# flysoaryun/LF-VIO

Measured on AMD Instinct MI355X. Metric: sliding-window solves/sec (10 KF x N landmarks), higher is better.
Workload: dtype f64; 1 GPU; window300; landmarks=300, observations=1419, windows_per_gpu=1, marginalization=MARGIN_OLD, parallelism=1 independent window stream(s), one per GPU, no data-path collective

## Files before the change

### lf-vio_amd/csrc/dev_types.h

```cpp
#pragma once
#include "../../include/lfvio.h"

constexpr int KC = 73;
constexpr int KP = 172;
constexpr int WLD = 80;
__host__ __device__ inline int w_row_len(int cnt) { return 6 * cnt + 9; }
constexpr int COL_B = 73;
constexpr int COL_K = 74;
constexpr int NQ = 105;
constexpr int NG = 210;
constexpr int NGP = 212;
constexpr int NPAIR = 121;
constexpr int NT = 15;
constexpr int SCHUR_LEN = NT * 256;
constexpr int PACKED = KP * (KP + 1) / 2;
constexpr int JMAX_SWEEPS = 20;
constexpr int PRE_CHUNK_LIMIT = 2 * 121;
constexpr int SUM_ITEMS_CAP = PRE_CHUNK_LIMIT * 209 + 64;
constexpr int SUM_VIS_PACKED = 73 * 74 / 2, SUM_VIS = SUM_VIS_PACKED + 73;
constexpr int HPP_CAP = 16384;
constexpr int XOFF_H = 0;
constexpr int XOFF_G = 14880;
constexpr int XOFF_S = XOFF_G + 176;
constexpr int XOFF_C = XOFF_S + 15 * 256;
constexpr int XCH_LEN = XOFF_C + 16;
constexpr int XP_WGS = 128, XOFF_P = XCH_LEN, XCH_ALLOC = XCH_LEN + 2 * XP_WGS;
enum { XS_COST = 0, XS_G2, XS_ASV2, XS_LAM2, XS_BMAX, XS_GN2, XS_GGN, XS_CCOST, XS_MLIN, XS_MQUAD, XS_DN, XS_XN, XS_N0, XS_ERR };
constexpr int LM_BLOCK = 64;
constexpr int CHUNK_LANES = 64;
constexpr int CHUNK_MAX = 64;
constexpr int SCHUR_LM = 64;
constexpr int LMS = 16;
constexpr int IMU_RAW = 450 + 16;
constexpr int IMU_OUT = 900 + 30 + 2;

__host__ __device__ inline int off_pose(int f) { return 6 * f; }
__host__ __device__ inline int off_ex() { return 66; }
__host__ __device__ inline int off_td() { return 72; }
__host__ __device__ inline int off_sb(int f) { return 73 + 9 * f; }
__host__ __device__ inline int pidx(int i, int j) { return i >= j ? i * (i + 1) / 2 + j : j * (j + 1) / 2 + i; }

struct FrameState {
  double pose[LFVIO_NUM_FRAMES][7];
  double sb[LFVIO_NUM_FRAMES][9];
  double ex[7];
  double td;
};

struct Tab {
  double R[11][9], P[11][3];
  double ric[9], ricT[9], tic[3];
  double M1[11][9];
  double M2[NPAIR][9];
  double T[NPAIR][9];
  double c[NPAIR][3];
};
constexpr int TAB_EX_BIT = 11;
constexpr double TAB_OFF_SPHERE = 1e-14;
__host__ __device__ inline int tab_cj(int pair) { return (pair % 11) * 11 + pair / 11; }

enum {
  Q_GG = 0,
  Q_GN,
  Q_NN,
  Q_gG,
  Q_gN,
  Q_GRAD_SQ,
  Q_GN_SQ,
  Q_GRAD_GN,
  Q_ZG,
  Q_LGN,
  Q_LGG,
  Q_LEX,
  Q_COUNT = 16
};

#ifndef LFVIO_SPEC_EXTRA
#define LFVIO_SPEC_EXTRA 3
#endif
constexpr int SPEC_EXTRA = LFVIO_SPEC_EXTRA, SPEC_MAX_LM = 320;
constexpr int WT_PAIRS = (KC + 1) / 2;
constexpr int SPEC_OWN = 72;
enum { SPEC_FREE = 0, SPEC_SIDE = 1, SPEC_MAIN = 2, SPEC_COMMIT = 3, SPEC_ABANDON = 4 };
enum { FIN_OPEN = 0, FIN_CLOSING = 1, FIN_MAIN = 2, FIN_SIDE = 3 };
constexpr int MAIL_MAX_LM = 8192;
#define TR_HEAD_FIELDS \
  double radius, mu, x_cost, x_norm, cand_cost, model_cost_change, dogleg_step_norm, alpha; \
  double cg, cn; \
  double gn_sq_total, grad_sq_total, grad_gn_total; \
  double step_sq_pose; \
  double xn2_pose_cand; \
  double gmax_pose, lm_bmax; \
  double initial_cost; \
  double function_tolerance; \
  double q[Q_COUNT]; \
  int iteration, cur, do_lin, do_schur, done, termination, chol_fail, scaled; \
  int num_succ, num_unsucc, consec_invalid, trace_len, step_valid, skip_step, error, new_point; \
  int spec_n, gn_unconfirmed;  \
  double cgE[SPEC_EXTRA], cnE[SPEC_EXTRA], snE[SPEC_EXTRA], step_sqE[SPEC_EXTRA], xn2E[SPEC_EXTRA];
struct TRHead {
  TR_HEAD_FIELDS
};
// ... 156 lines not shown
```

### lf-vio_amd/csrc/kernels_lin.h

```cpp
#pragma once
#include "dev_factors.h"
#include "kernels_spec.h"
#include "tr_decide.h"
#include <type_traits>

#define SLOT(base, stride) ((Slot *)((char *)(base) + (size_t)blockIdx.y * (stride)))

constexpr int MODE_SOLVE = 0;
constexpr int MODE_MARG = 1;
constexpr int MODE_GATED = 16;
constexpr int MODE_DECIDE = 64;
constexpr int MODE_NOCOUNT = 32;
DEV bool tail_gate(const Slot *S, int done) { return done && S->tail_state == TAIL_OPEN; }
DEV bool is_marg(int mode) { return mode >= MODE_MARG; }
DEV const MargPlan *marg_plan(const Slot *S, int mode) { return &S->marg[mode - MODE_MARG]; }

DEV int gidx20(int p, int q) { return p * 20 - (p * (p - 1)) / 2 + (q - p); }

constexpr int SETUP_PRIOR_WGS = 16;
constexpr int SETUP_WGS = 2 + SETUP_PRIOR_WGS;
constexpr int SETUP_TILED_MAXN = 88;
__global__ __launch_bounds__(256, 4) void k_setup(char *base, size_t stride, int mode, int zero_wt) {
  Slot *S = SLOT(base, stride);
  const int tid = threadIdx.x;
  constexpr int SETUP_PRIOR_SLAB = 2048, SETUP_LDS = LFVIO_WINDOW_SIZE * 15 * 16;
  static_assert(SETUP_LDS >= SETUP_PRIOR_SLAB + LFVIO_MAX_PRIOR_DIM && SETUP_LDS >= 84 + TAB_SCRATCH, "k_setup's workspace");
  __shared__ double sh_setup[SETUP_LDS];
  const int setup_wgs = (zero_wt & 4) ? 3 : SETUP_WGS;
  if (blockIdx.x == 0) {
    const double *src = (const double *)&S->x0;
    double *dst = (double *)&S->x[0];
    for (int k = tid; k < (int)(sizeof(FrameState) / 8); k += 256) dst[k] = src[k];
    if (tid == 0) {
      TRState *t = &S->tr;
      tr_init(t, S->init_radius, S->fn_tol);
      S->tail_state = TAIL_OPEN;
      S->passes_used = 0;
      S->dec_pending = 0;
      if (mode >= MODE_MARG) t->mu = 0.0;
    }
    double *bt = sh_setup;
    if (tid < 77) bt[tid] = (&S->x0.pose[0][0])[tid];
    else if (tid < 84) bt[tid] = S->x0.ex[tid - 77];
    __syncthreads();
    const unsigned offm = build_tab(bt, &S->tab[0], tid, bt + 84);
    if (tid == 0) S->ex_fixed_off = ((offm >> TAB_EX_BIT) & 1u) && !S->est_ex;
    if (tid == 0 && S->spec_on) spec_arm(S);
  } else if (blockIdx.x == 1) {
    if (tid >= 16 * ((LFVIO_WINDOW_SIZE + 3) & ~3)) return;
    const int grp = tid >> 4, l = tid & 15;
    const int f = grp < LFVIO_WINDOW_SIZE ? grp : 0;
    const bool mine = grp < LFVIO_WINDOW_SIZE && S->imu_active[f];
    const double *cov = S->imu[f].covariance;
    double m0[15], m1[15];
#pragma unroll
    for (int r = 0; r < 15; r++) {
      m0[r] = l < 15 ? cov[r * 15 + l] : (r == 0 ? 1.0 : 0.0);
      m1[r] = r == l + 1 ? 1.0 : 0.0;
    }
#pragma unroll
    for (int k = 0; k < 15; k++) {
      int p = k;
      double best = -1.0, piv = 0.0;
#pragma unroll
      for (int r = 0; r < 15; r++) {
        const double v = fabs(m0[r]);
        if (r >= k && v > best) best = v, p = r, piv = m0[r];
      }
      p = row_bcast_ik(p, k), piv = row_bcast_k(piv, k);
      double csr[15];
#pragma unroll
      for (int r = 0; r < 15; r++) csr[r] = row_bcast_k(m0[r], k);
      const double ck = csr[k];
#pragma unroll
      for (int r = 0; r < 15; r++) csr[r] = r == p ? ck : csr[r];
      auto step = [&](double(&m)[15]) {
        double Mp = m[0];
#pragma unroll
        for (int r = 1; r < 15; r++) Mp = p == r ? m[r] : Mp;
        const double Mk = m[k], mk = Mp / piv;
#pragma unroll
        for (int r = 0; r < 15; r++) {
          const double Msr = r == p ? Mk : m[r];
          m[r] = r == k ? mk : Msr - csr[r] * mk;
        }
      };
      step(m0), step(m1);
    }
    double *T = sh_setup + f * (15 * 16);
// ... 196 lines not shown
  int rows = Nlim - lm0;
  rows = rows > lmb ? lmb : rows;
  auto sweep = [&](auto ntl) {
    constexpr int NTL = decltype(ntl)::value;
    for (int s4 = 0; 4 * s4 < rows; s4++) {
      const int row = 4 * s4 + kk;
      const double coef = lcoef[row], eb = le[row];
#pragma unroll
      for (int j = 0; j < NTL; j++)
        acc[j] = __builtin_amdgcn_mfma_f64_16x16x4f64(coef * tile[row][ct[j]], tile[row][cu[j]] * (scale_k[j] ? eb : 1.0), acc[j], 0, 0, 0);
    }
  };
  if (TIGHT) {
    if (__builtin_amdgcn_readfirstlane(wv) + 12 < NT) sweep(std::integral_constant<int, 4>{});
    else sweep(std::integral_constant<int, 3>{});
  } else {
    for (int s4 = 0; 4 * s4 < rows; s4++) {
      const int row = 4 * s4 + kk;
      const double coef = lcoef[row], eb = le[row];
#pragma unroll
      for (int j = 0; j < 4; j++) {
        if (wv + 4 * j >= NT) continue;
        const double xa = tile[row][ct[j]];
        double xb = tile[row][cu[j]];
        if (mode == MODE_SOLVE && cu[j] == COL_K) xb *= eb;
        acc[j] = __builtin_amdgcn_mfma_f64_16x16x4f64(coef * xa, xb, acc[j], 0, 0, 0);
      }
    }
  }
#pragma unroll
  for (int j = 0; j < 4; j++) {
    if (wv + 4 * j >= NT) continue;
#pragma unroll
    for (int r = 0; r < 4; r++) part[(wv + 4 * j) * 256 + r * 64 + lane] = acc[j][r];
  }
}
DEV int w_col(int ci, int start, int cnt) { return ci < 6 * cnt ? 6 * start + ci : 66 + (ci - 6 * cnt); }

struct LinView {
  const FrameState *x;
  const Tab *tab;
  const double *lam;
  double mu;
};

template <int LPT>
DEV void lin_schur_only_role(Slot *S, const LinView &lv, int wg, double *lds, double *part) {
  constexpr int LMB = LIN_THREADS / LPT;
  double(*tile)[WLD + 1] = (double(*)[WLD + 1]) lds;
  double *lcoef = lds + LM_BLOCK * (WLD + 1) + 64, *le = lcoef + LM_BLOCK;
  const int tid = threadIdx.x;
  for (int e = tid; e < LM_BLOCK * (WLD + 1); e += LIN_THREADS) lds[e] = 0.0;
  __syncthreads();
  {
    const int lml = tid / LPT, q = tid % LPT, l = wg * LMB + lml;
    if (l < S->N) {
      const int st = S->lm_start[l], cnt = S->lm_cnt[l];
      const double *w = S->W + S->lm_woff[l];
      for (int ci = q; ci < w_row_len(cnt); ci += LPT) tile[lml][w_col(ci, st, cnt)] = w[ci];
    }
  }
  if (tid < LM_BLOCK) {
    const int l = wg * LMB + tid;
    double cf = 0.0, eb = 0.0;
    if (tid < LMB && l < S->N) {
      const double sc = S->scale_l[l], s2a = sc * sc * S->a[l];
      const double D2 = fmin(fmax(s2a, 1e-6), 1e32);
      eb = s2a + lv.mu * D2;
      const double einv = 1.0 / eb;
      cf = sc * sc * einv;
      S->einv_l[l] = einv;
    }
    lcoef[tid] = cf, le[tid] = eb;
  }
  __syncthreads();
  schur_block<false>(wg * LMB, LMB, MODE_SOLVE, S->N, tile, lcoef, le, part);
}

#ifdef LFVIO_LIN_PROFILE
#define LSTAMP(k) do { if (blockIdx.x == 0 && mode == MODE_SOLVE && threadIdx.x == 0) S->dbg[k] = (long long)__builtin_readcyclecounter(); } while (0)
#else
#define LSTAMP(k) do { } while (0)
#endif
template <bool TIGHT, int LPT, bool OFFS>
DEV void lin_landmark_role(Slot *S, const LinView &lv, int wg, int mode, double *lds, double *part) {
  constexpr int LMB = LIN_THREADS / LPT;
  double(*tile)[WLD + 1] = (double(*)[WLD + 1]) lds;
  double *red = lds + LM_BLOCK * (WLD + 1);
  double *lcoef = red + 64, *le = lcoef + LM_BLOCK;
  const int tid = threadIdx.x, lml = tid / LPT, q = tid % LPT;
  const TRState *tr = &S->tr;
  const Tab *T = lv.tab;
  const int Nlim = is_marg(mode) ? marg_plan(S, mode)->N0 : S->N;
  const int l = wg * LMB + lml;
  const bool valid = l < Nlim;
  const int est_td = S->est_td;
  const int est_ex = is_marg(mode) ? 1 : S->est_ex;
  const double td = lv.x->td;
  LSTAMP(22);
  for (int e = tid; e < LM_BLOCK * (WLD + 1); e += LIN_THREADS) lds[e] = 0.0;
  if (tid < 2 * LM_BLOCK) lcoef[tid] = 0.0;
  __syncthreads();
  LSTAMP(8);
  double a = 0, b = 0, cost = 0, lam = 1.0, wtd = 0;
  d3 wPi = mk3(0, 0, 0), wTi = wPi, wTic = wPi, wTx = wPi;
  int i = 0, cnt_l = 0, woff_l = 0;
  if (valid) {
    i = S->lm_start[l];
    const int k = S->lm_cnt[l], o0 = S->lm_obs0[l];
    cnt_l = k, woff_l = S->lm_woff[l];
    lam = lv.lam[l];
    ObsPair ob;
    load_obs(S, o0, ob.pi, ob.vi, ob.tdi, ob.rowi);
    const m33 ricT = ldm(T->ricT);
    const unsigned offm = OFFS ? tab_offmask(T) : 0u;
    for (int o = 1 + q; o < k; o += LPT) {
      const int j = i + o, pair = i * 11 + j;
      load_obs(S, o0 + o, ob.pj, ob.vj, ob.tdj, ob.rowj);
      PairU u;
      if (OFFS) load_pair_uniform(T, pair, offm, u);
      else load_pair_uniform(T, pair, u);
      Basis B;
      visual_basis<OFFS>(ob, lam, td, est_td, S->tr_over_row, S->half_row, S->sqrt_info, u, B);
      const double jl0 = B.jl[0], jl1 = B.jl[1];
      d3 eR = jl0 * B.red[0] + jl1 * B.red[1];
      const m33 M1 = ldm(T->M1[j]);
      d3 wp = vmul(eR, M1);
      wPi = wPi + wp;
      wTi = wTi + (jl0 * B.jti[0] + jl1 * B.jti[1]);
      d3 wtj = jl0 * B.jtj[0] + jl1 * B.jtj[1];
      tile[lml][6 * j + 0] = -wp.x, tile[lml][6 * j + 1] = -wp.y, tile[lml][6 * j + 2] = -wp.z;
      tile[lml][6 * j + 3] = wtj.x, tile[lml][6 * j + 4] = wtj.y, tile[lml][6 * j + 5] = wtj.z;
      m33 M3 = u.M2;
#pragma unroll
      for (int e = 0; e < 9; e++) M3.a[e] -= ricT.a[e];
      wTic = wTic + vmul(eR, M3);
      wTx = wTx + (jl0 * B.jtx[0] + jl1 * B.jtx[1]);
      wtd += jl0 * B.jtd[0] + jl1 * B.jtd[1];
      a += jl0 * jl0 + jl1 * jl1;
      b += jl0 * B.r[0] + jl1 * B.r[1];
      cost += 0.5 * B.rho0;
    }
  }
  LSTAMP(9);
  wPi = track_sum3<LPT>(wPi), wTi = track_sum3<LPT>(wTi), wTic = track_sum3<LPT>(wTic), wTx = track_sum3<LPT>(wTx);
  wtd = track_sum<LPT>(wtd), a = track_sum<LPT>(a), b = track_sum<LPT>(b), cost = track_sum<LPT>(cost);
  const bool lead = valid && q == 0;
  if (lead) {
    tile[lml][6 * i + 0] = wPi.x, tile[lml][6 * i + 1] = wPi.y, tile[lml][6 * i + 2] = wPi.z;
    tile[lml][6 * i + 3] = wTi.x, tile[lml][6 * i + 4] = wTi.y, tile[lml][6 * i + 5] = wTi.z;
    if (est_ex) {
      tile[lml][66] = wTic.x, tile[lml][67] = wTic.y, tile[lml][68] = wTic.z;
      tile[lml][69] = wTx.x, tile[lml][70] = wTx.y, tile[lml][71] = wTx.z;
    }
    if (est_td) tile[lml][72] = wtd;
  }
  double g2 = 0, asv2 = 0, lam2 = 0, bmax = 0;
  if (lead) {
    double s = 1.0, D2 = a;
    if (mode == MODE_SOLVE) {
      if (!tr->scaled) {
        s = 1.0 / (1.0 + sqrt(a));
        S->scale_l[l] = s;
      } else {
        s = S->scale_l[l];
      }
      D2 = fmin(fmax(s * s * a, 1e-6), 1e32);
      const double dg = sqrt(D2);
      const double gr = s * b / dg;
      S->diag_l[l] = dg;
      S->grad_l[l] = gr;
      g2 = gr * gr;
      const double v = gr / dg;
      asv2 = s * s * a * v * v;
      tile[lml][COL_K] = b / D2;
      const double s2a = s * s * a;
      const double eb = s2a + lv.mu * D2, einv = 1.0 / eb;
      le[lml] = eb, lcoef[lml] = s * s * einv;
      S->einv_l[l] = einv;
    } else {
      const double cf = (a > 1e-8) ? 1.0 / a : 0.0;
      le[lml] = a, lcoef[lml] = cf;
      S->einv_l[l] = cf;
    }
    S->a[l] = a;
    S->b[l] = b;
    tile[lml][COL_B] = b;
    lam2 = lam * lam;
    bmax = fabs(b);
  } else {
    cost = 0.0;
  }
  LSTAMP(18);
  cost = wave_sum(cost);
  g2 = wave_sum(g2);
  asv2 = wave_sum(asv2);
  lam2 = wave_sum(lam2);
  bmax = wave_max(bmax);
  if ((tid & 63) == 0) {
    double *r = red + 8 * (tid >> 6);
    r[0] = cost, r[1] = g2, r[2] = asv2, r[3] = lam2, r[4] = bmax;
  }
  lds_barrier();
  if (tid < 5) {
    double *p = S->lm_part + (size_t)(LPT == 8 ? wg >> 1 : wg) * LMS + (LPT == 8 && (wg & 1) ? 10 : 0);
    p[tid] = tid < 4 ? ((red[tid] + red[8 + tid]) + (red[16 + tid] + red[24 + tid]))
                     : fmax(fmax(red[4], red[12]), fmax(red[20], red[28]));
  }
  LSTAMP(19);
  if (valid) {
    double *w = S->W + woff_l;
    for (int ci = q; ci < w_row_len(cnt_l); ci += LPT) w[ci] = tile[lml][w_col(ci, i, cnt_l)];
  }
  if (TIGHT && mode == MODE_SOLVE && S->N <= SPEC_MAX_LM) {
    constexpr int WGRP = LIN_THREADS / LMB;
    const int lr = tid % LMB, wg4 = tid / LMB;
    double2 *wt = (double2 *)(double *)S->Wt + wg * LMB + lr;
    constexpr int WPT = (WT_PAIRS + WGRP - 1) / WGRP;
    double2 v[WPT];
#pragma unroll
    for (int k = 0; k < WPT; k++) {
      const int cp = wg4 + WGRP * k, c = cp < WT_PAIRS ? 2 * cp : 0;
      v[k] = make_double2(tile[lr][c], c + 1 < KC ? tile[lr][c + 1] : 0.0);
    }
#pragma unroll
    for (int k = 0; k < WPT; k++) {
      const int cp = wg4 + WGRP * k;
      if (cp < WT_PAIRS) wt[(size_t)cp * SPEC_MAX_LM] = v[k];
    }
  }
  LSTAMP(23);
  schur_block<TIGHT>(wg * LMB, LMB, mode, Nlim, tile, lcoef, le, part);
  LSTAMP(20);
}

template <bool OFFS>
DEV void lin_gram_role(Slot *S, const LinView &lv, int wg, int mode, double *lds) {
  const int wv = threadIdx.x >> 6, lane = threadIdx.x & 63;
  const int chunk = 4 * wg + wv;
  if (chunk >= S->nChunks) return;
  if (is_marg(mode) && chunk >= marg_plan(S, mode)->nChunks0) return;
  double *my = lds + wv * (32 * 17 + 256 + 14 * 20);
  double(*stage)[17] = (double(*)[17]) my;
  double(*Qf)[16] = (double(*)[16])(my + 32 * 17);
  double(*E)[20] = (double(*)[20])(my + 32 * 17 + 256);
  double(*T1)[20] = (double(*)[20]) my;
  const Tab *T = lv.tab;
  const int pair = S->chunk_pair[chunk];
  const int j = pair % 11;
  const int begin = S->chunk_begin[chunk], end = S->chunk_end[chunk];
  const int est_td = S->est_td;
  const double td = lv.x->td;
  PairU u;
  if (OFFS) load_pair_uniform(T, pair, tab_offmask(T), u);
  else load_pair_uniform(T, pair, u);
  for (int e = lane; e < 14 * 20; e += 64) E[0][e] = 0.0;
  for (int e = lane; e < 32 * 17; e += 64) stage[0][e] = 0.0;
  const int idx = begin + lane;
  double c0[14], c1[14];
#pragma unroll
  for (int e = 0; e < 14; e++) c0[e] = c1[e] = 0.0;
  if (idx < end) {
    const int oj = S->pm_obs[idx], l = S->pm_lm[idx];
    const int oi = S->lm_obs0[l];
    const double lam = lv.lam[l];
    ObsPair ob;
    load_obs(S, oi, ob.pi, ob.vi, ob.tdi, ob.rowi);
    load_obs(S, oj, ob.pj, ob.vj, ob.tdj, ob.rowj);
    Basis B;
    visual_basis<OFFS>(ob, lam, td, est_td, S->tr_over_row, S->half_row, S->sqrt_info, u, B);
    c0[0] = B.red[0].x, c0[1] = B.red[0].y, c0[2] = B.red[0].z;
    c1[0] = B.red[1].x, c1[1] = B.red[1].y, c1[2] = B.red[1].z;
    c0[3] = B.jti[0].x, c0[4] = B.jti[0].y, c0[5] = B.jti[0].z;
    c1[3] = B.jti[1].x, c1[4] = B.jti[1].y, c1[5] = B.jti[1].z;
    c0[6] = B.jtj[0].x, c0[7] = B.jtj[0].y, c0[8] = B.jtj[0].z;
    c1[6] = B.jtj[1].x, c1[7] = B.jtj[1].y, c1[8] = B.jtj[1].z;
    c0[9] = B.jtx[0].x, c0[10] = B.jtx[0].y, c0[11] = B.jtx[0].z;
    c1[9] = B.jtx[1].x, c1[10] = B.jtx[1].y, c1[11] = B.jtx[1].z;
    c0[12] = B.jtd[0], c1[12] = B.jtd[1];
    c0[13] = B.r[0], c1[13] = B.r[1];
  }
  double4_t acc = double4_t{0, 0, 0, 0};
  const int nrounds = (end - begin + 15) >> 4;
  for (int r = 0; r < nrounds; r++) {
    __builtin_amdgcn_fence(__ATOMIC_RELEASE, "wavefront");
    if ((lane >> 4) == r) {
      const int row = 2 * (lane & 15);
#pragma unroll
      for (int e = 0; e < 14; e++) stage[row][e] = c0[e], stage[row + 1][e] = c1[e];
    }
    __builtin_amdgcn_fence(__ATOMIC_ACQ_REL, "wavefront");
#pragma unroll
    for (int g = 0; g < 8; g++) {
      const double v = stage[4 * g + (lane >> 4)][lane & 15];
      acc = __builtin_amdgcn_mfma_f64_16x16x4f64(v, v, acc, 0, 0, 0);
    }
  }
  __builtin_amdgcn_fence(__ATOMIC_RELEASE, "wavefront");
#pragma unroll
  for (int r = 0; r < 4; r++) Qf[(lane >> 4) + 4 * r][lane & 15] = acc[r];
  if (lane < 9) {
    const int r = lane / 3, c = lane % 3;
    const double m1 = T->M1[j][lane];
    E[r][c] = m1;
    E[r][6 + c] = -m1;
    E[r][12 + c] = T->M2[pair][lane] - T->ricT[lane];
  } else if (lane < 12) {
    const int k = lane - 9;
    E[3 + k][3 + k] = 1.0;
    E[6 + k][9 + k] = 1.0;
    E[9 + k][15 + k] = 1.0;
  } else if (lane == 12) {
    E[12][18] = 1.0;
    E[13][19] = 1.0;
  }
  __builtin_amdgcn_fence(__ATOMIC_ACQ_REL, "wavefront");
  for (int e = lane; e < 14 * 20; e += 64) {
    const int r = e / 20, c = e % 20;
    double s = 0;
#pragma unroll
    for (int k = 0; k < 14; k++) s = fma(Qf[r][k], E[k][c], s);
    T1[r][c] = s;
  }
  __builtin_amdgcn_fence(__ATOMIC_ACQ_REL, "wavefront");
  double *out = S->gram_part + (size_t)chunk * NGP;
  for (int e = lane; e < 400; e += 64) {
    const int p = e / 20, c = e % 20;
    if (p > c) continue;
    double s = 0;
#pragma unroll
    for (int k = 0; k < 14; k++) s = fma(E[k][p], T1[k][c], s);
    out[gidx20(p, c)] = s;
  }
}

template <bool raw_ready>
DEV void lin_imu_role(Slot *S, const LinView &lv, int f, int mode, double *lds) {
  double(*Jr)[30] = (double(*)[30]) lds;
  double(*Jw)[31] = (double(*)[31])(lds + 450);
  double *rr = lds + 450 + 465, *rw = rr + 16;
  const int tid = threadIdx.x;
  double *out = S->imu_out + (size_t)f * IMU_OUT;
  const bool active = S->imu_active[f] && (mode == MODE_SOLVE || (f == 0 && marg_plan(S, mode)->use_imu0)) &&
                      (!S->sharded || S->pose_side);
  if (!active) {
    for (int e = tid; e < IMU_OUT; e += LIN_THREADS) out[e] = 0.0;
    return;
  }
  const FrameState *x = lv.x;
  if (raw_ready) {
    const double *raw = S->imu_raw + (size_t)f * IMU_RAW;
    for (int e = tid; e < 450; e += LIN_THREADS) Jr[e / 30][e % 30] = raw[e];
    if (tid < 15) rr[tid] = raw[450 + tid];
  } else {
    for (int e = tid; e < 450; e += LIN_THREADS) Jr[e / 30][e % 30] = 0.0;
    __syncthreads();
    if (tid == 0) imu_raw_residual(&S->imu[f], S->g, x->pose[f], x->sb[f], x->pose[f + 1], x->sb[f + 1], rr);
    if (tid == 64) imu_raw_jacobian(&S->imu[f], S->g, x->pose[f], x->sb[f], x->pose[f + 1], x->sb[f + 1], &Jr[0][0]);
  }
  __syncthreads();
  const double *Sq = S->imu_sqrt[f];
  if (tid < 15) {
    double s = 0;
    for (int k = 0; k < 15; k++) s = fma(Sq[tid * 15 + k], rr[k], s);
    rw[tid] = s;
  }
  for (int e = tid; e < 450; e += LIN_THREADS) {
    const int r = e / 30, c = e % 30;
    double s = 0;
    for (int k = r; k < 15; k++) s = fma(Sq[r * 15 + k], Jr[k][c], s);
    Jw[r][c] = s;
  }
  __syncthreads();
  for (int e = tid; e < 900; e += LIN_THREADS) {
    const int p = e / 30, c = e % 30;
    double s = 0;
#pragma unroll
    for (int k = 0; k < 15; k++) s = fma(Jw[k][p], Jw[k][c], s);
    out[e] = s;
  }
  if (tid < 30) {
    double s = 0;
#pragma unroll
    for (int k = 0; k < 15; k++) s = fma(Jw[k][tid], rw[k], s);
    out[900 + tid] = s;
  }
  if (tid == 32) {
    double s = 0;
    for (int k = 0; k < 15; k++) s = fma(rw[k], rw[k], s);
    out[930] = 0.5 * s;
  }
}

template <bool STAGED>
DEV void lin_prior_role(Slot *S, const LinView &lv, int mode, double *lds) {
  const int n = S->prior_n;
  const bool staged = STAGED && n <= LIN_PRIOR_N;
  double *Js = lds, *dx = lds + (STAGED ? LIN_PRIOR_N * LIN_PRIOR_N : 0), *r = dx + KP, *part = r + KP;
  const int tid = threadIdx.x;
  double *g = S->prior_g;
  for (int c = tid; c < KP + 4; c += LIN_THREADS) g[c] = 0.0;
  if (!S->prior_valid || (S->sharded && !S->pose_side)) return;
  const FrameState *x = lv.x;
  const double *Jg = S->prior_J;
  if (staged) {
    constexpr int PER = (LIN_PRIOR_N * LIN_PRIOR_N + LIN_THREADS - 1) / LIN_THREADS;
    double v[PER];
#pragma unroll
    for (int k = 0; k < PER; k++) v[k] = tid + LIN_THREADS * k < n * n ? Jg[tid + LIN_THREADS * k] : 0.0;
    if (tid < S->prior_nb) prior_block_dx(S, x, tid, dx);
#pragma unroll
    for (int k = 0; k < PER; k++)
      if (tid + LIN_THREADS * k < n * n) Js[tid + LIN_THREADS * k] = v[k];
  } else if (tid < S->prior_nb) {
    prior_block_dx(S, x, tid, dx);
  }
  __syncthreads();
  const double *J = staged ? Js : Jg;
  for (int row = tid >> 2; row < n; row += LIN_THREADS / 4) {
    double s = 0;
    for (int c = tid & 3; c < n; c += 4) s = fma(J[row * n + c], dx[c], s);
    s = quad_sum(s);
    if ((tid & 3) == 0) r[row] = S->prior_r[row] + s;
  }
  __syncthreads();
  {
    const int c = tid & 127, h = tid >> 7, k0 = h ? n / 2 : 0, k1 = h ? n : n / 2;
    for (int cc = c; cc < n; cc += 128) {
      double s = 0;
      for (int k = k0; k < k1; k++) s = fma(J[k * n + cc], r[k], s);
      part[h * KP + cc] = s;
    }
  }
  __syncthreads();
  for (int c = tid; c < n; c += LIN_THREADS) g[S->prior_cmap[c]] = part[c] + part[KP + c];
  if (tid < 64) {
    double cs = 0;
    for (int row = tid; row < n; row += 64) cs += r[row] * r[row];
    cs = wave_sum(cs);
    if (tid == 0) g[KP] = 0.5 * cs;
  }
}

__global__ __launch_bounds__(64) void k_imu_raw(char *base, size_t stride, int count) {
  const int g = blockIdx.x * 64 + threadIdx.x;
  if (g >= count * LFVIO_WINDOW_SIZE) return;
  const int slot = g / LFVIO_WINDOW_SIZE, f = g - slot * LFVIO_WINDOW_SIZE;
  Slot *S = reinterpret_cast<Slot *>(base + stride * (size_t)slot);
  const TRFlags fl = tr_flags(&S->tr);
  if (fl.done | !fl.do_lin) return;
  if (!S->imu_active[f] || (S->sharded && !S->pose_side)) return;
  const FrameState *x = &S->x[fl.cur];
  double *raw = S->imu_raw + (size_t)f * IMU_RAW;
  for (int e = 0; e < 450; e++) raw[e] = 0.0;
  imu_raw_residual(&S->imu[f], S->g, x->pose[f], x->sb[f], x->pose[f + 1], x->sb[f + 1], raw + 450);
  imu_raw_jacobian(&S->imu[f], S->g, x->pose[f], x->sb[f], x->pose[f + 1], x->sb[f + 1], raw);
}

constexpr int LIN_ROLE_LM = 1, LIN_ROLE_GRAM = 2, LIN_ROLE_POSE = 4, LIN_ROLE_ALL = 7;
constexpr int LIN_ROLE_POSE_RAW = 8;
constexpr int LIN_LDS_POSE = 1024;
template <int ROLES, bool OFFS = true>
__global__ __launch_bounds__(LIN_THREADS, ROLES == LIN_ROLE_GRAM ? 3 : (ROLES == LIN_ROLE_POSE_RAW ? 6 : 2)) void k_lin(char *base, size_t stride, int mode_bits, int gLw, int gCh) {
  Slot *S = SLOT(base, stride);
  TRState *tr = &S->tr;
  const int mode = mode_bits & (MODE_GATED - 1);
  LSTAMP(21);
  const TRFlags fl = tr_flags(tr);
  int do_lin = fl.do_lin, do_schur = fl.do_schur, cur = fl.cur, acc_z = 0;
  double mu = tr->mu;
  int num_succ = tr->num_succ;
  if (mode_bits & MODE_GATED) {
    if (!tail_gate(S, fl.done)) return;
  } else {
    int done = fl.done;
    const bool owner = blockIdx.x == 0 && !(mode_bits & MODE_NOCOUNT);
    if ((mode_bits & MODE_DECIDE) && !done) {
      __shared__ TRDecision dsh;
      if (threadIdx.x < 64) {
        TRHead t = *reinterpret_cast<const TRHead *>(tr);
        const int K = decide_candidates(t);
        DecideSums sm;
        decide_sums(S, t, K, 0, S->nLmBlocks, threadIdx.x, sm);
        if (threadIdx.x == 0) {
          const int az = decide_walk(t, sm, K, 0, S->max_iter, owner ? tr : nullptr);
          decision_from(dsh, t, az);
          if (owner) S->dec = dsh, S->dec_pending = 1;
        }
      }
      __syncthreads();
      do_lin = __builtin_amdgcn_readfirstlane(dsh.do_lin), do_schur = __builtin_amdgcn_readfirstlane(dsh.do_schur);
      cur = __builtin_amdgcn_readfirstlane(dsh.cur), acc_z = __builtin_amdgcn_readfirstlane(dsh.acc_z), done = __builtin_amdgcn_readfirstlane(dsh.done);
      num_succ = __builtin_amdgcn_readfirstlane(dsh.num_succ);
      mu = __hiloint2double(__builtin_amdgcn_readfirstlane(__double2hiint(dsh.mu)), __builtin_amdgcn_readfirstlane(__double2loint(dsh.mu)));
      if (acc_z > 0 && blockIdx.x == gridDim.x - 1 && !(mode_bits & MODE_NOCOUNT)) {
        copy_accepted(S, acc_z, cur, S->N, threadIdx.x, LIN_THREADS);
        if (S->spec_on) {
          __threadfence();
          __syncthreads();
          if (threadIdx.x == 0) spec_publish(S, num_succ, cur);
        }
      } else if (acc_z == 0 && owner && threadIdx.x == 0 && S->spec_on) spec_publish(S, num_succ, cur);
    } else if (owner && threadIdx.x == 0 && mode == MODE_SOLVE && S->spec_on) spec_publish(S, num_succ, cur);
    if (mode == MODE_SOLVE && owner && !done && threadIdx.x == 0) S->passes_used++;
    if (done | (!do_lin & !do_schur)) return;
  }
  LinView lv;
  lv.x = acc_z > 0 ? &S->xE[acc_z > 0 ? acc_z - 1 : 0] : &S->x[cur];
  lv.tab = acc_z > 0 ? &S->tabE[acc_z > 0 ? acc_z - 1 : 0] : &S->tab[cur];
  lv.lam = acc_z > 0 ? (const double *)S->lamE[acc_z > 0 ? acc_z - 1 : 0] : (const double *)S->lam[cur];
  lv.mu = mu;
  __shared__ __attribute__((aligned(16))) double lds[(ROLES & (LIN_ROLE_LM | LIN_ROLE_GRAM)) ? LIN_LDS : LIN_LDS_POSE];
  int b = blockIdx.x;
  if (b < gLw) {
    if (ROLES & LIN_ROLE_LM) {
      const int half = S->lm_half, lmb = half ? LM_BLOCK / 2 : LM_BLOCK;
      const int nblk = ((is_marg(mode) ? marg_plan(S, mode)->N0 : S->N) + lmb - 1) / lmb;
      if (b >= nblk) return;
      double *part = S->schur_part + (size_t)b * SCHUR_LEN;
      if (half) {
        if (do_lin) lin_landmark_role<ROLES == LIN_ROLE_ALL, 8, OFFS>(S, lv, b, mode, lds, part);
        else lin_schur_only_role<8>(S, lv, b, lds, part);
      } else {
        if (do_lin) lin_landmark_role<ROLES == LIN_ROLE_ALL, 4, OFFS>(S, lv, b, mode, lds, part);
        else lin_schur_only_role<4>(S, lv, b, lds, part);
      }
    }
    return;
  }
  if (!do_lin) return;
  b -= gLw;
  if (b < gCh) {
    if (ROLES & LIN_ROLE_GRAM) lin_gram_role<OFFS>(S, lv, b, mode, lds);
    return;
  }
  b -= gCh;
  if (ROLES & (LIN_ROLE_POSE | LIN_ROLE_POSE_RAW)) {
    if (b < LFVIO_WINDOW_SIZE) {
      if (ROLES & LIN_ROLE_POSE_RAW) lin_imu_role<true>(S, lv, b, mode, lds);
      else lin_imu_role<false>(S, lv, b, mode, lds);
      return;
    }
    lin_prior_role<ROLES == LIN_ROLE_ALL>(S, lv, mode, lds);
  }
}

DEV int schur_index(int R, int Cc) {
  const int t = R >> 4, u = Cc >> 4;
  const int tile = t * 5 - (t * (t - 1)) / 2 + (u - t);
  const int row = R & 15, col = Cc & 15;
  return tile * 256 + (row >> 2) * 64 + ((row & 3) << 4) + col;
}

constexpr int HPP_ITEMS = PACKED + KP;
constexpr int HPP_BLOCKS = (HPP_ITEMS + 255) / 256;

DEV int imu_local(int c, int f) {
  if (c < 66) {
    const int fr = c / 6, l = c - 6 * fr;
    if (fr == f) return l;
    if (fr == f + 1) return 15 + l;
    return -1;
  }
  if (c < KC) return -1;
  const int fr = (c - KC) / 9, l = (c - KC) - 9 * fr;
  if (fr == f) return 6 + l;
  if (fr == f + 1) return 21 + l;
  return -1;
}
DEV int col_frame(int c) { return c < 66 ? c / 6 : (c < KC ? -10 : (c - KC) / 9); }
DEV bool pose_terms_here(const Slot *S, int r) { return !S->sharded || S->pose_side == 1 || (S->pose_side == 2 && r >= KC); }

DEV bool col_active(const Slot *S, int c, int mode) {
  if (mode >= MODE_MARG) return true;
  if (!S->est_ex && c >= off_ex() && c < off_ex() + 6) return false;
  if (!S->est_td && c == off_td()) return false;
  return true;
}

constexpr int PRE_GROUP = 32;
__global__ __launch_bounds__(256) void k_presum(char *base, size_t stride, int mode_bits, int groups) {
  const int PRE_SCHUR_BLOCKS = (SCHUR_LEN / 256) * groups;
  Slot *S = SLOT(base, stride);
  const TRState *tr = &S->tr;
  const int mode = mode_bits & (MODE_GATED - 1);
  const TRFlags fl = tr_flags_decided(S);
  if (mode_bits & MODE_GATED) {
    if (!tail_gate(S, fl.done)) return;
  } else if (fl.done | (!fl.do_lin & !fl.do_schur)) return;
  const int tid = threadIdx.x;
  int b = blockIdx.x;
  if (b < NPAIR) {
    if (!fl.do_lin) return;
    const int chunk_limit = is_marg(mode) ? marg_plan(S, mode)->nChunks0 : S->nChunks;
    const int c0 = S->pair_chunk0[b];
    int c1 = S->pair_chunk0[b + 1];
    if (c1 > chunk_limit) c1 = chunk_limit;
    if (tid < NGP) {
      const double *gp = S->gram_part + tid;
      double s0 = 0, s1 = 0, s2 = 0, s3 = 0;
      int c = c0;
      for (; c + 4 <= c1; c += 4) {
        s0 += gp[(size_t)c * NGP], s1 += gp[(size_t)(c + 1) * NGP];
        s2 += gp[(size_t)(c + 2) * NGP], s3 += gp[(size_t)(c + 3) * NGP];
      }
      for (; c < c1; c++) s0 += gp[(size_t)c * NGP];
      S->pairG[(size_t)b * NGP + tid] = (s0 + s1) + (s2 + s3);
    }
    return;
  }
  b -= NPAIR;
  if (b < PRE_SCHUR_BLOCKS) {
    if (!fl.do_schur) return;
    const int grp = b / (SCHUR_LEN / 256), e = (b % (SCHUR_LEN / 256)) * 256 + tid;
    int parts = S->nSchurParts;
    if (is_marg(mode)) parts = (marg_plan(S, mode)->N0 + S->schur_lm - 1) / S->schur_lm;
    const int p0 = grp * PRE_GROUP;
    if (p0 >= parts) return;
    const int p1 = min(parts, p0 + PRE_GROUP);
    double *sp = S->schur_part + e;
    double a0 = 0, a1 = 0, a2 = 0, a3 = 0;
    int p = p0;
    for (; p + 4 <= p1; p += 4) {
      a0 += sp[(size_t)p * SCHUR_LEN], a1 += sp[(size_t)(p + 1) * SCHUR_LEN];
      a2 += sp[(size_t)(p + 2) * SCHUR_LEN], a3 += sp[(size_t)(p + 3) * SCHUR_LEN];
    }
    for (; p < p1; p++) a0 += sp[(size_t)p * SCHUR_LEN];
    sp[(size_t)p0 * SCHUR_LEN] = (a0 + a1) + (a2 + a3);
    return;
  }
  if (!fl.do_lin) return;
  __shared__ double red[5][256];
  const int blocks = S->nLmBlocks;
  double v[5] = {0, 0, 0, 0, 0};
  for (int k = tid; k < blocks; k += 256) {
    const double *q = S->lm_part + (size_t)k * LMS;
    v[0] += q[0], v[1] += q[1], v[2] += q[2], v[3] += q[3], v[4] = fmax(v[4], q[4]);
  }
#pragma unroll
  for (int k = 0; k < 5; k++) red[k][tid] = v[k];
  __syncthreads();
  for (int w = 128; w > 0; w >>= 1) {
    if (tid < w) {
#pragma unroll
      for (int k = 0; k < 4; k++) red[k][tid] += red[k][tid + w];
      red[4][tid] = fmax(red[4][tid], red[4][tid + w]);
    }
    __syncthreads();
  }
  if (tid < 5) S->lm_sum[tid] = red[tid][0];
}

struct SumArgs {
  long long sum_off, sum_end_marg, sum_items, gram_part, pairG, imu_out, prior_A;
};
template <class T>
DEV T *blob_at(const Slot *S, long long off) { return (T *)((char *)S + off); }
#define SUM_KEEP(v) asm volatile("" ::"v"(v))

DEV void sum_hpp_entry(Slot *S, const SumArgs &o, int mode_bits, int e) {
  const int mode = mode_bits & (MODE_GATED - 1);
  const bool in = e < HPP_ITEMS;
  const int ec = in ? e : 0;
  const bool packed = ec < PACKED;
  int r, c;
  if (packed) {
    r = (int)((sqrt(8.0 * ec + 1.0) - 1.0) * 0.5);
    while ((r + 1) * (r + 2) / 2 <= ec) r++;
    while (r * (r + 1) / 2 > ec) r--;
    c = ec - r * (r + 1) / 2;
  } else {
    r = c = ec - PACKED;
  }
  const TRFlags fl = tr_flags_decided(S);
  const int tail_state = S->tail_state, est_ex = S->est_ex, est_td = S->est_td, prior_valid = S->prior_valid, sharded = S->sharded;
  const int pose_side = S->pose_side, pre_gram = S->pre_gram, prior_n = S->prior_n;
  const int marg_chunks = is_marg(mode) ? marg_plan(S, mode)->nChunks0 : 1;
  const int vis = r < KC ? (packed ? ec : SUM_VIS_PACKED + r) : 0;
  const int beg = blob_at<int>(S, o.sum_off)[vis];
  int end = blob_at<int>(S, o.sum_off)[vis + 1];
  const int endm = blob_at<int>(S, o.sum_end_marg)[vis];
  const int pr = S->prior_inv[r], pc = S->prior_inv[c];
  const double pg = S->prior_g[r];
  double imu_v[2] = {0.0, 0.0};
  const int f0 = col_frame(r);
  const double *imu_out = blob_at<double>(S, o.imu_out);
#pragma unroll
  for (int u = 0; u < 2; u++) {
    const int f = f0 - 1 + u;
    if (f0 >= 0 && f >= 0 && f < LFVIO_WINDOW_SIZE) {
      const int pl = imu_local(r, f), ql = imu_local(c, f);
      if (packed) {
        if (pl >= 0 && ql >= 0) imu_v[u] = imu_out[(size_t)f * IMU_OUT + pl * 30 + ql];
      } else if (pl >= 0) {
        imu_v[u] = imu_out[(size_t)f * IMU_OUT + 900 + pl];
      }
    }
  }
  SUM_KEEP(beg);
  SUM_KEEP(end);
  SUM_KEEP(endm);
  SUM_KEEP(pr);
  SUM_KEEP(pc);
  SUM_KEEP(pg);
  SUM_KEEP(imu_v[0]);
  SUM_KEEP(imu_v[1]);
  if (mode_bits & MODE_GATED) {
    if (!(fl.done && tail_state == TAIL_OPEN)) return;
  } else if (fl.done | !fl.do_lin) return;
  if (!in) return;
  const bool act_r = is_marg(mode) || !((!est_ex && r >= off_ex() && r < off_ex() + 6) || (!est_td && r == off_td()));
  const bool act_c = is_marg(mode) || !((!est_ex && c >= off_ex() && c < off_ex() + 6) || (!est_td && c == off_td()));
  double val = 0.0;
  if (act_r && act_c) {
    if (is_marg(mode)) end = marg_chunks > 0 ? endm : beg;
    const bool pterms = !sharded || pose_side == 1 || (pose_side == 2 && r >= KC);
    const bool use_prior = packed && prior_valid && pterms && pr >= 0 && pc >= 0;
    double pa = 0.0;
    if (use_prior) pa = blob_at<double>(S, o.prior_A)[pr * prior_n + pc];
    if (r < KC) {
      const int *it = blob_at<int>(S, o.sum_items);
      const double *gp = blob_at<double>(S, pre_gram ? o.pairG : o.gram_part);
      double s0 = 0, s1 = 0, s2 = 0, s3 = 0;
      int k = beg;
      for (; k + 4 <= end; k += 4) {
        const int o0 = it[k], o1 = it[k + 1], o2 = it[k + 2], o3 = it[k + 3];
        s0 += gp[o0], s1 += gp[o1], s2 += gp[o2], s3 += gp[o3];
      }
      for (; k < end; k++) s0 += gp[it[k]];
      val += (s0 + s1) + (s2 + s3);
    }
    if (packed) {
      if (f0 >= 0 && pterms) {
#pragma unroll
        for (int u = 0; u < 2; u++) {
          const int f = f0 - 1 + u;
          if (f >= 0 && f < LFVIO_WINDOW_SIZE && imu_local(r, f) >= 0 && imu_local(c, f) >= 0) val += imu_v[u];
        }
      }
      if (use_prior) val += pa;
// ... 104 lines not shown
```

### lf-vio_amd/csrc/kernels_linw.h

```cpp
#pragma once
#include "kernels_lin.h"

#ifdef LFVIO_LINW_PROFILE
#ifndef LFVIO_LINB_GROUP
#define LFVIO_LINB_GROUP 0
#endif
#define WSTAMP(k) do { if (blockIdx.y == 0 && threadIdx.x == 0) S->dbg[k] = (long long)__builtin_readcyclecounter(); } while (0)
#define WACC(k, t0) do { wacc[(k) - 24] += (long long)__builtin_readcyclecounter() - (t0); } while (0)
#define WNOW() ((long long)__builtin_readcyclecounter())
#else
#define WSTAMP(k) do { } while (0)
#define WACC(k, t0) do { } while (0)
#define WNOW() 0ll
#endif

constexpr int LW_THREADS = 256;
constexpr int LW_STAGE = 32 * 17;
constexpr int LW_WAVE = LW_STAGE + 256 + 64;
constexpr int LW_D = 0, LW_FX = 11 * 21, LW_XX = LW_FX + 11 * 42, LW_G = LW_XX + 28, LW_DUMMY = LW_G + 76;
constexpr int LW_PRIV = 800;
static_assert(LW_DUMMY < LW_PRIV, "private accumulator layout");
constexpr int LW_NPAIR = 55, LW_OFF = LW_NPAIR * 36;
constexpr int LW_PRIV0 = LINW_WAVES * LW_WAVE, LW_OFF0 = LW_PRIV0 + LINW_WAVES * LW_PRIV, LW_RED0 = LW_OFF0 + LW_OFF;
constexpr int LW_LDS_P1 = LW_RED0 + LINW_WAVES * 8;
// ... 328 lines not shown
  auto factor_on = [&](int f) { return S->imu_active[f] && pose_rank && (mode == MODE_SOLVE || (f == 0 && marg_plan(S, mode)->use_imu0)); };
  for (int e = lane; e < 3 * 16 * LW_JLD; e += 64) my[e] = 0.0;
  __builtin_amdgcn_fence(__ATOMIC_ACQ_REL, "wavefront");
  if (lane < 3) {
    const int f = wv + 4 * lane;
    if (f < LFVIO_WINDOW_SIZE && factor_on(f)) {
      double rr[15];
      imu_raw_residual(&S->imu[f], S->g, x->pose[f], x->sb[f], x->pose[f + 1], x->sb[f + 1], rr);
      double *Jr = Jr3 + 16 * LW_JLD * lane;
#pragma unroll
      for (int k = 0; k < 15; k++) Jr[k * LW_JLD + 30] = rr[k];
      imu_raw_jacobian(&S->imu[f], S->g, x->pose[f], x->sb[f], x->pose[f + 1], x->sb[f + 1], Jr, LW_JLD);
    }
  }
  __builtin_amdgcn_fence(__ATOMIC_ACQ_REL, "wavefront");
  WSTAMP(29);
  const int kq = lane >> 4, ii = lane & 15;
  double *imu_out = (double *)((char *)S + imu_off);
  double sa3[3][4];
#pragma unroll
  for (int q = 0; q < 3; q++) {
    const int f = wv + 4 * q < LFVIO_WINDOW_SIZE ? wv + 4 * q : 0;
    const double *Sq = S->imu_sqrt[f];
#pragma unroll
    for (int s4 = 0; s4 < 4; s4++) {
      const int k = 4 * s4 + kq;
      sa3[q][s4] = (ii < 15 && k < 15) ? Sq[ii * 15 + k] : 0.0;
    }
  }
#pragma unroll
  for (int q = 0; q < 3; q++) {
    const int f = wv + 4 * q;
    if (f >= LFVIO_WINDOW_SIZE) break;
    double *out = imu_out + (size_t)f * IMU_OUT;
    if (!factor_on(f)) {
      for (int e = lane; e < IMU_OUT; e += 64) out[e] = 0.0;
      continue;
    }
    const double(*Jr)[LW_JLD] = (const double(*)[LW_JLD])(Jr3 + 16 * LW_JLD * q);
    const double(&sa)[4] = sa3[q];
    double4_t w0 = double4_t{0, 0, 0, 0}, w1 = w0;
#pragma unroll
    for (int s4 = 0; s4 < 4; s4++) {
      w0 = __builtin_amdgcn_mfma_f64_16x16x4f64(sa[s4], Jr[4 * s4 + kq][ii], w0, 0, 0, 0);
      w1 = __builtin_amdgcn_mfma_f64_16x16x4f64(sa[s4], Jr[4 * s4 + kq][16 + ii], w1, 0, 0, 0);
    }
#pragma unroll
    for (int r = 0; r < 4; r++) Jw[kq + 4 * r][ii] = w0[r], Jw[kq + 4 * r][16 + ii] = w1[r];
    __builtin_amdgcn_fence(__ATOMIC_ACQ_REL, "wavefront");
    double4_t g00 = double4_t{0, 0, 0, 0}, g01 = g00, g11 = g00;
#pragma unroll
    for (int s4 = 0; s4 < 4; s4++) {
      const double v0 = Jw[4 * s4 + kq][ii], v1 = Jw[4 * s4 + kq][16 + ii];
      g00 = __builtin_amdgcn_mfma_f64_16x16x4f64(v0, v0, g00, 0, 0, 0);
      g01 = __builtin_amdgcn_mfma_f64_16x16x4f64(v0, v1, g01, 0, 0, 0);
      g11 = __builtin_amdgcn_mfma_f64_16x16x4f64(v1, v1, g11, 0, 0, 0);
    }
#pragma unroll
    for (int r = 0; r < 4; r++) {
      const int row = kq + 4 * r, c1 = 16 + ii;
      auto ord = [](int p) { return p < 6 ? p : p < 15 ? p + 6 : p < 21 ? p - 9 : p; };
      const int r2 = 16 + row;
      if (ord(row) >= ord(ii)) out[row * 30 + ii] = g00[r];
      if (c1 < 30) {
        if (ord(row) >= ord(c1)) out[row * 30 + c1] = g01[r];
        else out[c1 * 30 + row] = g01[r];
      } else if (c1 == 30) out[900 + row] = g01[r];
      if (r2 < 30) {
        if (c1 < 30) {
          if (ord(r2) >= ord(c1)) out[r2 * 30 + c1] = g11[r];
        } else if (c1 == 30) out[900 + r2] = g11[r];
      } else if (r2 == 30 && c1 == 30) out[930] = 0.5 * g11[r];
    }
    __builtin_amdgcn_fence(__ATOMIC_ACQ_REL, "wavefront");
  }
}

constexpr int LW_PRIOR_MAXN = 88;
static_assert(LW_PRIOR_MAXN * LW_PRIOR_MAXN + 4 * KP <= LW_LDS_P1, "prior stage fits");
DEV void linw_prior(Slot *S, const LinView &lv, double *lw) {
  const int tid = threadIdx.x;
  const int n = S->prior_n;
  if (!S->prior_valid || (S->sharded && !S->pose_side) || n > LW_PRIOR_MAXN) {
    lin_prior_role<false>(S, lv, MODE_SOLVE, lw);
    __syncthreads();
    return;
  }
  double *Js = lw, *dx = lw + LW_PRIOR_MAXN * LW_PRIOR_MAXN, *r = dx + KP, *part = r + KP;
  double *g = S->prior_g;
  const double *J = S->prior_J;
  const double r0_row = (tid >> 1) < n ? S->prior_r[tid >> 1] : 0.0;
  const int cmap_c = tid < n ? S->prior_cmap[tid] : 0;
  {
    constexpr int PJ = 8, ROUNDS = (LW_PRIOR_MAXN * LW_PRIOR_MAXN + PJ * LW_THREADS - 1) / (PJ * LW_THREADS);
    const int nn = n * n;
#pragma unroll 1
    for (int b = 0; b < ROUNDS && b * PJ * LW_THREADS < nn; b++) {
      double v[PJ];
#pragma unroll
      for (int k = 0; k < PJ; k++) {
        const int e = tid + LW_THREADS * (PJ * b + k);
        v[k] = J[e < nn ? e : 0];
      }
#pragma unroll
      for (int k = 0; k < PJ; k++) {
        const int e = tid + LW_THREADS * (PJ * b + k);
        if (e < nn) Js[e] = v[k];
      }
    }
  }
  for (int c = tid; c < KP + 4; c += LW_THREADS) g[c] = 0.0;
  if (tid < S->prior_nb) prior_block_dx(S, lv.x, tid, dx);
  __syncthreads();
  {
    const int row = tid >> 1, h = tid & 1;
    double s0 = 0, s1 = 0, s2 = 0, s3 = 0;
    if (row < n) {
      const double *jr = Js + row * n;
      int c = h;
      for (; c + 6 < n; c += 8) s0 = fma(jr[c], dx[c], s0), s1 = fma(jr[c + 2], dx[c + 2], s1), s2 = fma(jr[c + 4], dx[c + 4], s2), s3 = fma(jr[c + 6], dx[c + 6], s3);
      for (; c < n; c += 2) s0 = fma(jr[c], dx[c], s0);
    }
    double sum = (s0 + s1) + (s2 + s3);
    sum += dpp_f64<0xB1>(sum);
    if (row < n && h == 0) r[row] = r0_row + sum;
  }
  __syncthreads();
  {
    const int c = tid & 127, h = tid >> 7, k0 = h ? n / 2 : 0, k1 = h ? n : n / 2;
    if (c < n) {
      double s0 = 0, s1 = 0, s2 = 0, s3 = 0;
      int k = k0;
      for (; k + 3 < k1; k += 4)
        s0 = fma(Js[k * n + c], r[k], s0), s1 = fma(Js[(k + 1) * n + c], r[k + 1], s1), s2 = fma(Js[(k + 2) * n + c], r[k + 2], s2), s3 = fma(Js[(k + 3) * n + c], r[k + 3], s3);
      for (; k < k1; k++) s0 = fma(Js[k * n + c], r[k], s0);
      part[h * KP + c] = (s0 + s1) + (s2 + s3);
    }
  }
  __syncthreads();
  static_assert(LW_PRIOR_MAXN <= LW_THREADS, "one column per thread");
  if (tid < n) g[cmap_c] = part[tid] + part[KP + tid];
  if (tid < 64) {
    double cs = 0;
    for (int row = tid; row < n; row += 64) cs += r[row] * r[row];
    cs = wave_sum(cs);
    if (tid == 0) g[KP] = 0.5 * cs;
  }
  __syncthreads();
}

constexpr int LWT_ABS = 1 << 16, LWT_EX = 1 << 17, LWT_TD = 1 << 18;

template <bool OFFS>
DEV void linw_body(Slot *S, double *lw, const LinwArgs &A, int mode_bits) {
  TRState *tr = &S->tr;
  const int tid = threadIdx.x, wv = tid >> 6, lane = tid & 63;
  TRFlags fl = tr_flags(tr);
  const double mu = tr->mu;
  const int mode = mode_bits & (MODE_GATED - 1);
  const bool marg = is_marg(mode);
  const int N = marg ? marg_plan(S, mode)->N0 : S->N, est_ex = marg ? 1 : S->est_ex, est_td = marg ? 1 : S->est_td;
  if (marg) {
    if ((mode_bits & MODE_GATED) && !tail_gate(S, fl.done)) return;
    fl.do_lin = fl.do_schur = 1;
  } else {
    if (!fl.done && tid == 0) S->passes_used++;
    if (fl.done | (!fl.do_lin & !fl.do_schur)) return;
// ... 160 lines not shown
  double *einv_l = lw_at<double>(S, A.einv_l);
  const int nblk = (N + LM_BLOCK - 1) / LM_BLOCK;
  constexpr int WPT = (WT_PAIRS + 3) / 4;
  double2 wreg[WPT];
  double w_sc = 0, w_a = 0, w_b = 0;
  auto request = [&](int blk) {
    const int l = blk * LM_BLOCK + lane;
    const int pmin = 3 * rfl(blk_start[blk]);
#pragma unroll
    for (int k = 0; k < WPT; k++) {
      const int cp = wv + 4 * k;
      wreg[k] = (cp < WT_PAIRS && cp >= pmin && l < N) ? wt0[(size_t)cp * SPEC_MAX_LM + l] : make_double2(0.0, 0.0);
    }
    if (tid < LM_BLOCK && l < N) w_sc = scale_l[l], w_a = av[l], w_b = bv[l];
  };
  for (int e = tid; e < LM_BLOCK * 6; e += LW_THREADS) tile[e / 6][75 + e % 6] = 0.0;
  if (nblk > 0) request(0);
  for (int blk = 0; blk < nblk; blk++) {
    __syncthreads();
    {
      const int l = blk * LM_BLOCK + lane;
#pragma unroll
      for (int k = 0; k < WPT; k++) {
        const int cp = wv + 4 * k;
        if (cp < WT_PAIRS) {
          tile[lane][2 * cp] = wreg[k].x;
          if (2 * cp + 1 < KC) tile[lane][2 * cp + 1] = wreg[k].y;
        }
      }
      if (tid < LM_BLOCK) {
        double cf = 0.0, eb = 0.0, bl = 0.0, kap = 0.0;
        if (l < N && marg) {
          cf = (w_a > 1e-8) ? 1.0 / w_a : 0.0, eb = w_a, bl = w_b;
        } else if (l < N) {
          const double s2a = w_sc * w_sc * w_a;
          const double D2 = fmin(fmax(s2a, 1e-6), 1e32);
          eb = s2a + mu * D2;
          const double einv = 1.0 / eb;
          cf = w_sc * w_sc * einv;
          if (!fl.do_lin) einv_l[l] = einv;
          bl = w_b, kap = bl / D2;
        }
        lcoef[tid] = cf, le[tid] = eb;
        tile[tid][COL_B] = bl, tile[tid][COL_K] = kap;
      }
    }
    if (blk + 1 < nblk) request(blk + 1);
    __syncthreads();
    auto sweep = [&](auto ntl) {
      constexpr int NTL4 = decltype(ntl)::value;
#pragma unroll
      for (int s4 = 0; s4 < LM_BLOCK / 4; s4++) {
        const int row = 4 * s4 + kk;
        const double coef = lcoef[row], eb = le[row];
#pragma unroll
        for (int j = 0; j < NTL4; j++) {
          const double xa = tile[row][ct[j]];
          double xb = tile[row][cu[j]];
          if (scale_k[j]) xb *= eb;
          acc[j] = __builtin_amdgcn_mfma_f64_16x16x4f64(coef * xa, xb, acc[j], 0, 0, 0);
        }
      }
    };
    if (__builtin_amdgcn_readfirstlane(wv) + 12 < NT) sweep(std::integral_constant<int, 4>{});
    else sweep(std::integral_constant<int, 3>{});
  }
  WSTAMP(13);
  double *ss = lw_at<double>(S, A.schur_sum);
#pragma unroll
  for (int j = 0; j < 4; j++) {
    if (wv + 4 * j >= NT) continue;
#pragma unroll
    for (int r = 0; r < 4; r++) ss[(wv + 4 * j) * 256 + r * 64 + lane] = acc[j][r];
  }
  if (tid == 0 && !marg && fl.do_lin) S->wt_clean = 1;
  WSTAMP(14);
}
template <bool OFFS = true>
__global__ __launch_bounds__(LW_THREADS, 2) void k_linw(char *base, size_t stride, const LinwArgs A, int mode_bits) {
  extern __shared__ __attribute__((aligned(16))) double lw[];
  linw_body<OFFS>(SLOT(base, stride), lw, A, mode_bits);
}

constexpr int LINB_LEN = SUM_VIS + SCHUR_LEN + 8;
__global__ __launch_bounds__(256) void k_linb_gather(char *base, size_t stride) {
  Slot *S = SLOT(base, stride);
  if (!S->linw.big) return;
  const int i = blockIdx.x * 256 + threadIdx.x;
  if (i < S->N) {
    const int o = S->lm_obs0[i];
#pragma unroll
    for (int k = 0; k < 8; k++) S->anc[k][i] = S->obs[k][o];
  }
  if (i < S->NV) {
    const int o = S->pm_obs[i];
    double v[8];
#pragma unroll
    for (int k = 0; k < 8; k++) v[k] = S->obs[k][o];
#pragma unroll
    for (int k = 0; k < 8; k++) S->pmo[k][i] = v[k];
    int lo = 0, hi = NPAIR;
    while (hi - lo > 1) {
      const int mid = (lo + hi) >> 1;
      if (S->linw.pair_obs0[mid] <= i) lo = mid;
      else hi = mid;
    }
    S->pm_pair[i] = (unsigned char)lo;
  }
}
#ifdef LFVIO_LINW_PROFILE
#ifndef LFVIO_LINB_GROUP
#define LFVIO_LINB_GROUP 0
#endif
#define BSTAMP(k) do { if (blockIdx.x == LFVIO_LINB_GROUP && blockIdx.y == 0 && threadIdx.x == 0) S->dbg[k] = (long long)__builtin_readcyclecounter(); } while (0)
#else
#define BSTAMP(k) do { } while (0)
#endif
template <bool OFFS>
DEV void linb_body(Slot *S, double *lw, const LinwArgs &A) {
  TRState *tr = &S->tr;
  const int tid = threadIdx.x, wv = tid >> 6, lane = tid & 63;
  const TRFlags fl = tr_flags(tr);
  const double mu = tr->mu;
  const LinwPlan *P = &S->linw;
  const int ng = P->ng, g = blockIdx.x;
  if (g > ng) return;
  if (g == 0 && tid == 0 && !fl.done) S->passes_used++;
  if (fl.done | (!fl.do_lin & !fl.do_schur)) return;
  LinView lv;
  lv.x = &S->x[fl.cur], lv.tab = &S->tab[fl.cur], lv.lam = lw_at<const double>(S, A.lam[fl.cur]), lv.mu = mu;
  if (g == ng) {
    if (!fl.do_lin) return;
    linw_imu(S, lv, lw, A.imu_out, MODE_SOLVE);
    __syncthreads();
    linw_prior(S, lv, lw);
    return;
  }
  const int L0 = rfl(S->linb_lm0[g]), ns = rfl(S->linb_ns[g]), s = ns >> 16, L1 = L0 + (ns & 0xffff);
  const int est_ex = S->est_ex, est_td = S->est_td;
  double *out = lw_at<double>(S, A.part) + (size_t)g * LINB_LEN;
  if (fl.do_lin) {
    constexpr int P3_E = (SUM_VIS + LW_THREADS - 1) / LW_THREADS;
    int p3[P3_E];
#pragma unroll
    for (int q = 0; q < P3_E; q++) p3[q] = A.asm_tab[tid + LW_THREADS * q < SUM_VIS ? tid + LW_THREADS * q : 0];
    const int nstr = (L1 - L0 + LM_BLOCK - 1) / LM_BLOCK, split = nstr <= 1 ? 4 : nstr <= 2 ? 2 : 1;
    const int mine = wv / split + (lane == 1 ? 4 : 0);
    const int lm0w = L0 + LM_BLOCK * mine, nw = min(max(L1 - lm0w, 0), LM_BLOCK);
    const int kmaxw = nw > 0 ? S->lm_cnt[lm0w + nw - 1] : 0;
    const int nmine = (wv / split < nstr ? 1 : 0) + (wv / split + 4 < nstr ? 1 : 0);
    BSTAMP(8);
    for (int e = tid; e < LB_RED0 + LINW_WAVES * 8; e += LW_THREADS) lw[e] = 0.0;
    __syncthreads();
    BSTAMP(9);
    double part[5];
    linw_strips<true, OFFS>(S, lv, A, fl.cur, fl.scaled, MODE_SOLVE, lw, part, 0, nmine, lm0w, nw | (s << 8) | (kmaxw << 16), 1 + wv % split, split);
    if (lane == 0) {
#pragma unroll
      for (int k = 0; k < 5; k++) lw[LB_RED0 + 8 * wv + k] = part[k];
    }
    __syncthreads();
    BSTAMP(10);
#pragma unroll
    for (int q = 0; q < P3_E; q++) {
      const int e = tid + LW_THREADS * q, d = p3[q];
      int at = d & 0xffff;
      bool live = true;
// ... 246 lines not shown
```

### lf-vio_amd/csrc/kernels_marg.h

```cpp
#pragma once
#include "kernels_solve.h"

constexpr int MARG_THREADS = 768;
constexpr int MARG_MAXD = 96;
constexpr int LDN = 80;
constexpr double JACOBI_TOL = 1e-19;
constexpr size_t MARG_LDS = (size_t)19072 * sizeof(double);
constexpr int BT_GROUP = 4;

DEV void gauge_landmarks(Slot *S, int l0) {
  const int l = l0 + (int)threadIdx.x;
  double *lam = S->lam[S->tr.cur];
  if (l < S->N) lam[l] = 1.0 / (1.0 / lam[l]);
}
template <class T>
DEV void copy_rounds(T *dst, const T *src, int n, int tid, int nthr) {
  for (int k0 = tid; k0 < n; k0 += 8 * nthr) {
    T v[8];
#pragma unroll
    for (int q = 0; q < 8; q++) v[q] = src[k0 + q * nthr < n ? k0 + q * nthr : 0];
#pragma unroll
    for (int q = 0; q < 8; q++)
      if (k0 + q * nthr < n) dst[k0 + q * nthr] = v[q];
  }
// ... 118 lines not shown
  if (!tail_gate(S, S->tr.done)) return;
  const int spec = S->spec_on;
  if (spec) {
    if (threadIdx.x == 0) spec_closing(S);
    __syncthreads();
  }
  {
    constexpr int LT = (SPEC_MAX_LM + 127) / 128;
    double *lam = S->lam[S->tr.cur];
    const int N = S->N, tid = threadIdx.x;
    double lv[LT];
#pragma unroll
    for (int k = 0; k < LT; k++) lv[k] = lam[tid + 128 * k < N ? tid + 128 * k : 0];
#pragma unroll
    for (int k = 0; k < LT; k++)
      if (tid + 128 * k < N) lam[tid + 128 * k] = 1.0 / (1.0 / lv[k]);
    for (int l0 = 128 * LT; l0 < N; l0 += 128) gauge_landmarks(S, l0);
  }
  gauge_poses(S, 1, publish != 0);
  if (spec && threadIdx.x == 0) spec_settle(S);
}
DEV void gauge_poses(Slot *S, int gated, bool publish) {
  TRState *ts = &S->tr;
  const int tid = threadIdx.x;
  __shared__ double rot[9], P0[3], oP0[3];
  FrameState *x = &S->x[ts->cur];
  if (tid == 0) {
    const m33 Rs0 = q2R(q_from_pose(S->x0.pose[0]));
    const m33 R00 = q2R(q_from_pose(x->pose[0]));
    const double h0 = sqrt(Rs0.a[0] * Rs0.a[0] + Rs0.a[3] * Rs0.a[3]), h00 = sqrt(R00.a[0] * R00.a[0] + R00.a[3] * R00.a[3]);
    const double c0 = Rs0.a[0] / h0, s0 = Rs0.a[3] / h0, c00 = R00.a[0] / h00, s00 = R00.a[3] / h00;
    const double cyd = c0 * c00 + s0 * s00, syd = s0 * c00 - c0 * s00;
    m33 rd;
    rd.a[0] = cyd, rd.a[1] = -syd, rd.a[2] = 0;
    rd.a[3] = syd, rd.a[4] = cyd, rd.a[5] = 0;
    rd.a[6] = 0, rd.a[7] = 0, rd.a[8] = 1;
    const double sin1deg = 0.017452406437283512;
    if (h0 < sin1deg || h00 < sin1deg) rd = mm(Rs0, tr(R00));
    for (int k = 0; k < 9; k++) rot[k] = rd.a[k];
    for (int k = 0; k < 3; k++) P0[k] = x->pose[0][k], oP0[k] = S->x0.pose[0][k];
  }
  __syncthreads();
  const m33 rd = ldm(rot);
  d3 Psi = mk3(0, 0, 0), Vsi = Psi;
  q4 qn = q4{1, 0, 0, 0};
  if (tid < 11) {
    const m33 Rsi = mm(rd, q2R(qnormalized(q_from_pose(x->pose[tid]))));
    Psi = mul(rd, ld3(x->pose[tid]) - ld3(P0)) + ld3(oP0);
    Vsi = mul(rd, ld3(x->sb[tid]));
    qn = R2q(Rsi);
  } else if (tid == 11) {
    qn = R2q(q2R(q_from_pose(x->ex)));
  }
  __syncthreads();
  __shared__ double bt[84 + TAB_SCRATCH];
  if (tid < 11) {
    const double pn[7] = {Psi.x, Psi.y, Psi.z, qn.x, qn.y, qn.z, qn.w};
#pragma unroll
    for (int k = 0; k < 7; k++) x->pose[tid][k] = pn[k], bt[7 * tid + k] = pn[k];
    x->sb[tid][0] = Vsi.x, x->sb[tid][1] = Vsi.y, x->sb[tid][2] = Vsi.z;
  } else if (tid == 11) {
    x->ex[3] = qn.x, x->ex[4] = qn.y, x->ex[5] = qn.z, x->ex[6] = qn.w;
#pragma unroll
    for (int k = 0; k < 3; k++) bt[77 + k] = x->ex[k];
    bt[80] = qn.x, bt[81] = qn.y, bt[82] = qn.z, bt[83] = qn.w;
  }
  __syncthreads();
  if (publish) publish_solution(S);
  if (tid == 0) {
    if (!gated) ts->done = 0;
    ts->do_lin = 1;
    ts->do_schur = 1;
    ts->chol_fail = 0;
  }
  build_tab(bt, &S->tab[ts->cur], tid, bt + 84);
}

__global__ __launch_bounds__(64) void k_spec_wait(char *base) {
  Slot *S = (Slot *)base;
  if (threadIdx.x != 0) return;
  const long long t0 = wall_clock64();
  while (spec_peek(&S->tail_state) == TAIL_WORKER && wall_clock64() - t0 < 10 * SPEC_WAIT_TICKS) __builtin_amdgcn_s_sleep(8);
}
__global__ __launch_bounds__(128) void k_spec_begin(char *base, size_t back) {
  Slot *S = (Slot *)base;
  Slot *S0 = (Slot *)(base - back);
  const int tid = threadIdx.x;
  __shared__ int sh_word, sh_go;
  const long long t0 = wall_clock64();
  for (;;) {
    if (tid == 0) {
      int go = 0, w = 0;
      const int last = S->shadow.last_word;
      for (;;) {
        const int f = spec_peek(&S0->spec.fin);
        w = spec_peek(&S0->spec.word);
        if (w != 0) {
          const int st = spec_ep(f) == spec_ep(w) ? spec_fin_state(f) : FIN_OPEN;
          if (st != FIN_OPEN) break;
          if (w != last) {
            go = 1;
            break;
          }
        }
        if (wall_clock64() - t0 > SPEC_WAIT_TICKS) break;
        __builtin_amdgcn_s_sleep(8);
      }
      spec_acquire();
      sh_word = w, sh_go = go;
    }
    __syncthreads();
    int go = __builtin_amdgcn_readfirstlane(sh_go);
    const int w = __builtin_amdgcn_readfirstlane(sh_word);
    if (!go) {
      if (tid == 0) S->shadow.word = 0, S->tr.done = 0;
      return;
    }
    const int ep = spec_ep(w), a = spec_acc(w), cur = w & 1;
    if (S->shadow.hdr_ep != ep) {
      const long long *src = (const long long *)S0;
      long long *dst = (long long *)S;
      constexpr int W0 = (int)(offsetof(Slot, lm_start) / 8), W1 = (int)(offsetof(Slot, x) / 8);
      static_assert(offsetof(Slot, lm_start) % 8 == 0 && offsetof(Slot, x) % 8 == 0, "header words");
      for (int k = tid; k < W1; k += 128) dst[k] = src[k] - (k >= W0 ? (long long)back : 0ll);
      const double *is = &S0->imu_sqrt[0][0];
      double *id = &S->imu_sqrt[0][0];
      for (int k = tid; k < LFVIO_WINDOW_SIZE * 225; k += 128) id[k] = is[k];
    }
    __syncthreads();
    {
      constexpr int XW = (int)(sizeof(FrameState) / 8), TW = (int)(sizeof(TRHead) / 8), XT = (XW + 127) / 128, LT = (SPEC_MAX_LM + 127) / 128;
      static_assert(TW <= 128, "the trust-region header in one trip");
      const double *xs = (const double *)&S0->x[cur];
      double *xd = (double *)&S->x[0];
      const double *ls = S0->lam[cur];
      double *ld = S->lam[0];
      const int N = S0->N;
      const long long *ts = (const long long *)&S0->tr;
      long long *td = (long long *)&S->tr;
      double xv[XT], lv[LT];
#pragma unroll
      for (int k = 0; k < XT; k++) xv[k] = xs[tid + 128 * k < XW ? tid + 128 * k : 0];
#pragma unroll
      for (int k = 0; k < LT; k++) lv[k] = ls[tid + 128 * k < N ? tid + 128 * k : 0];
      const long long tv = ts[tid < TW ? tid : 0];
#pragma unroll
      for (int k = 0; k < XT; k++)
        if (tid + 128 * k < XW) xd[tid + 128 * k] = xv[k];
#pragma unroll
      for (int k = 0; k < LT; k++)
        if (tid + 128 * k < N) ld[tid + 128 * k] = 1.0 / (1.0 / lv[k]);
      if (tid < TW) td[tid] = tv;
      for (int k = tid + 128 * LT; k < N; k += 128) ld[k] = 1.0 / (1.0 / ls[k]);
    }
    __syncthreads();
    if (tid == 0) {
      const int f = spec_ld(&S0->spec.fin), w2 = spec_ld(&S0->spec.word);
      const bool open = spec_ep(f) != ep || spec_fin_state(f) == FIN_OPEN;
      sh_go = (w2 == w && open && spec_cas(&S0->spec.own[a], SPEC_FREE, SPEC_SIDE) == SPEC_FREE) ? 1 : 0;
      S->shadow.hdr_ep = ep;
      S->shadow.last_word = w;
    }
    __syncthreads();
    go = __builtin_amdgcn_readfirstlane(sh_go);
    if (!go) {
      __syncthreads();
      continue;
    }
    if (tid == 0) {
      S->shadow.word = w, S->shadow.ticket = S0->spec.ticket;
      S->spec_on = 0, S->dec_pending = 0, S->tail_state = TAIL_OPEN, S->chain_err = 0;
      S->tr.cur = 0, S->tr.done = 1;
    }
    __syncthreads();
    break;
  }
  gauge_poses(S, 1, false);
}

DEV bool spd_inverse_wave(const double *Am, double *Xout, int m, int lane, double floor) {
  double a[15];
#pragma unroll
  for (int j = 0; j < 15; j++) a[j] = (lane < m && j < m) ? Am[lane * m + j] : (lane == j ? 1.0 : 0.0);
  bool ok = true;
  double dinv = 1.0;
#pragma unroll
  for (int j = 0; j < 15; j++) {
    const double d = readlane_f64(a[j], j);
    ok = ok && (d > 0.0);
    const double rs = fast_rsqrt(d);
    const double l = lane == j ? d * rs : a[j] * rs;
    a[j] = l;
    dinv = lane == j ? rs : dinv;
#pragma unroll
    for (int c = j + 1; c < 15; c++) a[c] = fma(-l, readlane_f64(l, c), a[c]);
  }
  double y[15];
#pragma unroll
  for (int i = 0; i < 15; i++) {
    double t = lane == i ? 1.0 : 0.0;
#pragma unroll
    for (int k = 0; k < i; k++) t = fma(-readlane_f64(a[k], i), y[k], t);
    y[i] = t * readlane_f64(dinv, i);
  }
  double fro = 0;
#pragma unroll
  for (int r = 0; r < 15; r++) {
    double x = 0;
#pragma unroll
    for (int i = r; i < 15; i++) x = fma(readlane_f64(y[i], r), y[i], x);
    if (lane < m && r < m) Xout[r * m + lane] = x, fro += x * x;
  }
  fro = wave_sum(fro);
  return ok && fro * floor * floor < 1.0;
}

DEV void rr_pair(int k, int step, int np, int n, int &p, int &q) {
  if (k == 0) {
    p = step, q = np - 1;
  } else {
    p = step + k;
    if (p >= np - 1) p -= np - 1;
    q = step - k;
    if (q < 0) q += np - 1;
  }
  if (q >= n) q = -1;
}
// ... 784 lines not shown
```

### lf-vio_amd/csrc/lfvio_hip.hip

```cpp
#include <hip/hip_runtime.h>
#include <dlfcn.h>
typedef struct ncclComm *ncclComm_t;
#define NCCL_UNIQUE_ID_BYTES 128
typedef struct {
  char internal[NCCL_UNIQUE_ID_BYTES];
} ncclUniqueId;
typedef int ncclResult_t;
typedef int ncclDataType_t;
typedef int ncclRedOp_t;
constexpr ncclResult_t ncclSuccess = 0;
constexpr ncclRedOp_t ncclSum = 0;
constexpr ncclDataType_t ncclDouble = 8;

#include <algorithm>
#include <chrono>
#include <cmath>
#include <cstdio>
#include <cstdlib>
#include <cstring>
#include <memory>
#include <string>
#include <type_traits>
#include <vector>

#include "../../include/lfvio.h"
#include "../../include/lfvio_debug.h"
#include "kernels_marg.h"
#include "kernels_solve.h"
#include "kernels_feat.h"
#include "kernels_linw.h"
#include "linb_plan.h"
#include "call_state.h"
#include "kernels_stepw.h"
#include "kernels_relo.h"
#include "kernels_twoview.h"
#include "kernels_vialign.h"
#include "kernels_pnp.h"

#define HIPCHK(ctx, call)                                                                      \
  do {                                                                                         \
    hipError_t e_ = (call);                                                                    \
    if (e_ != hipSuccess) {                                                                    \
      (ctx)->err = std::string(#call) + ": " + hipGetErrorString(e_);                          \
      return LFVIO_ERR_DEVICE;                                                                 \
    }                                                                                          \
  } while (0)

namespace {

inline size_t align_up(size_t v, size_t a) { return (v + a - 1) / a * a; }

struct Layout {
  int maxN = 0, maxM = 0;
  int capLmBlocks = 0, capChunks = 0, capSchurParts = 0;
  size_t in_begin = 0, in_end = 0, total = 0;
  size_t anc[8], pmo[8], pm_pair, linb_lm0, linb_ns, linw_begin = 0, linw_end = 0;
  size_t lm_start, lm_cnt, lm_obs0, lm_perm, lm_woff, lam0, obs[8], pm_obs, pm_lm, chunk_pair, chunk_begin, chunk_end, sum_off, sum_end_marg, sum_items, prior_J,
      prior_r;
  size_t lam[2], lamE[SPEC_EXTRA], cost_partE, prior_A, a, b, W, Wt, scale_l, grad_l, gn_l, diag_l, einv_l, d1, d2, gram_part, pairG, schur_part,
      xch, lm_part, cost_part, imu_out, imu_raw, mscr, eig_aux;
};

Layout make_layout(int maxN, int maxM) {
  Layout L;
  L.maxN = maxN;
  L.maxM = maxM;
  L.capLmBlocks = std::max(1, (maxN + LM_BLOCK - 1) / LM_BLOCK);
  L.capChunks = 64 + maxM / CHUNK_MAX;
  L.capSchurParts = std::max(L.capLmBlocks + 1, 2 * ((std::min(maxN, SPEC_MAX_LM) + LM_BLOCK - 1) / LM_BLOCK));
  static_assert(LINB_LEN >= SCHUR_LEN, "the Schur partials of k_lin share the array of k_linb's group partials, which are the larger");
  size_t o = align_up(sizeof(Slot), 256);
  auto take = [&](size_t bytes) {
    size_t r = o;
    o = align_up(o + bytes, 256);
    return r;
  };
  const size_t N = std::max(maxN, 1), M = std::max(maxM, 1), LB = (size_t)L.capLmBlocks * LM_BLOCK;
  L.in_begin = o;
  L.lm_start = take(N * 4), L.lm_cnt = take(N * 4), L.lm_obs0 = take(N * 4), L.lm_perm = take(N * 4);
  L.lm_woff = take((N + 1) * 4);
  L.lam0 = take(N * 8);
  for (int k = 0; k < 8; k++) L.obs[k] = take(M * 8);
  L.pm_obs = take(M * 4), L.pm_lm = take(M * 4);
  L.chunk_pair = take((size_t)L.capChunks * 4), L.chunk_begin = take((size_t)L.capChunks * 4),
  L.chunk_end = take((size_t)L.capChunks * 4);
  L.prior_r = take(LFVIO_MAX_PRIOR_DIM * 8);
  L.sum_off = take((size_t)(SUM_VIS + 1) * 4), L.sum_end_marg = take((size_t)SUM_VIS * 4);
  L.sum_items = take((size_t)SUM_ITEMS_CAP * 4);
  L.prior_J = take((size_t)LFVIO_MAX_PRIOR_DIM * LFVIO_MAX_PRIOR_DIM * 8);
  L.in_end = o;
  L.linw_begin = o;
  for (int k = 0; k < 8; k++) L.anc[k] = take(N * 8);
  for (int k = 0; k < 8; k++) L.pmo[k] = take(M * 8);
  L.pm_pair = take(M);
  L.linb_lm0 = take(((size_t)L.capLmBlocks + LFVIO_NUM_FRAMES + 1) * 4), L.linb_ns = take(((size_t)L.capLmBlocks + LFVIO_NUM_FRAMES + 1) * 4);
  L.linw_end = o;
  L.lam[0] = take(LB * 8), L.lam[1] = take(LB * 8);
  for (int k = 0; k < SPEC_EXTRA; k++) L.lamE[k] = take((size_t)SPEC_MAX_LM * 8);
  L.cost_partE = take((size_t)SPEC_EXTRA * (SPEC_MAX_LM / 64) * LMS * 8);
  L.prior_A = take((size_t)LFVIO_MAX_PRIOR_DIM * LFVIO_MAX_PRIOR_DIM * 8);
  L.a = take(LB * 8), L.b = take(LB * 8), L.W = take(LB * WLD * 8);
  L.Wt = take((size_t)WT_PAIRS * std::max((size_t)SPEC_MAX_LM, LB) * 16);
  L.scale_l = take(LB * 8), L.grad_l = take(LB * 8), L.gn_l = take(LB * 8), L.diag_l = take(LB * 8);
  L.einv_l = take(LB * 8), L.d1 = take(LB * 8), L.d2 = take(LB * 8);
  L.gram_part = take((size_t)L.capChunks * NGP * 8);
  L.pairG = take((size_t)NPAIR * NGP * 8);
  L.schur_part = take((size_t)L.capSchurParts * LINB_LEN * 8);
  L.xch = take((size_t)XCH_ALLOC * 8);
  L.lm_part = take((size_t)L.capLmBlocks * LMS * 8);
  L.cost_part = take((size_t)L.capLmBlocks * LMS * 8);
  L.imu_out = take((size_t)LFVIO_WINDOW_SIZE * IMU_OUT * 8);
  L.imu_raw = take((size_t)LFVIO_WINDOW_SIZE * IMU_RAW * 8);
  L.mscr = take((size_t)HPP_CAP * 8);
  L.eig_aux = take(4096);
  L.total = align_up(o, 4096);
  return L;
}

size_t down_bytes(int maxN) { return sizeof(FrameState) * 2 + sizeof(TRState) + 2 * ((size_t)maxN * 8 + 128) + sizeof(LfvioPrior) + 4096; }

struct SlotHostInfo {
  bool spec_on = false;
  bool offs_first = false, offs_all = false;
  int N = 0, M = 0, gLm = 0, gLw = 0, gCh = 0, gSc = 0;
  int marg_n = 0;
  int prior_n = 0;
  int max_iter = 0;
  double max_seconds = -1.0;
  std::vector<int> perm;
  bool linw_ok = false;
  bool linb_ok = false;
  int linb_ng = 0;
  bool uploaded = false;
  bool resident = false;
  LfvioPrior in_prior;
  bool has_in_prior = false;
  bool in_prior_device = false;
  struct MargOut {
    int valid = 0, n = 0, m = 0, nb = 0;
    int kind[LFVIO_MAX_PRIOR_BLOCKS], frame[LFVIO_MAX_PRIOR_BLOCKS], idx[LFVIO_MAX_PRIOR_BLOCKS];
  } marg_out[2];
  int mail_seq = 0;
  std::vector<int> list_key;
  int list_items = -1;
};

struct Grid {
  int lm, ch, sc, lw;
  int ch_raw;
};

struct SetupLaunch {
  int gx, bits;
};

struct Route {
  enum Sweep { ROLES = 0, LINW = 1, LINB = 2 } sweep;
  int count;
  Grid g;
  size_t role_wgs;
  bool split;
  int linb_gx;
  SetupLaunch setup;
  int offs;
};

struct GraphKey {
  int count = 0, lm = 0, ch = 0, sc = 0, sweep = -1, linb_gx = 0, offs = 0, setup = -1, spec = 0, passes = 0;
  bool operator==(const GraphKey &o) const {
    return count == o.count && lm == o.lm && ch == o.ch && sc == o.sc && sweep == o.sweep && linb_gx == o.linb_gx && offs == o.offs &&
           setup == o.setup && spec == o.spec && passes == o.passes;
  }
};

}

struct lfvio_ctx {
  int device = 0;
  hipStream_t stream = nullptr;
  char *d_feat = nullptr;
  size_t feat_bytes = 0;
  char *h_feat = nullptr;
  std::string err;
  int batch = 0;
  Layout L;
  char *d_base = nullptr;
  char *h_stage = nullptr;
  char *h_down = nullptr;
  size_t h_down_bytes = 0;
  std::vector<SlotHostInfo> info;
  std::vector<int> perm_build;
  hipGraphExec_t graph = nullptr;
  GraphKey graph_key;
  hipGraphExec_t chunk[2] = {}, tail[2][3] = {};
  hipGraphExec_t first[2][2][4][13] = {};
  int fixed_passes = 0;
  int recent_passes[4] = {0, 0, 0, 0}, recent_head = 0;
  int predict_passes = 4;
  double pass_seconds = 2e-4;
  GraphKey chunk_key;
// ... 753 lines not shown

template <class F>
int capture_graph(lfvio_ctx *c, hipStream_t stream, hipGraphExec_t *out, F &&enqueue) {
  hipGraph_t graph;
  HIPCHK(c, hipStreamBeginCapture(stream, hipStreamCaptureModeThreadLocal));
  CaptureGuard guard(stream);
  if (int rc = enqueue()) return rc;
  HIPCHK(c, guard.end(&graph));
  HIPCHK(c, hipGraphInstantiate(out, graph, nullptr, nullptr, 0));
  HIPCHK(c, hipGraphDestroy(graph));
  return LFVIO_OK;
}

constexpr int CH_BUCKET = 16;

Grid grid_for(lfvio_ctx *c, int count) {
  Grid g{1, 1, 1, 1, 1};
  for (int s = 0; s < count; s++) {
    g.ch_raw = std::max(g.ch_raw, c->info[s].gCh);
    g.lm = std::max(g.lm, c->info[s].gLm);
    g.lw = std::max(g.lw, c->info[s].gLw);
    g.ch = std::max(g.ch, c->info[s].gCh);
    g.sc = std::max(g.sc, c->info[s].gSc);
  }
  g.ch = (g.ch + CH_BUCKET - 1) / CH_BUCKET * CH_BUCKET;
  return g;
}

int slots_offs(const lfvio_ctx *c, int count) {
  int r = 0;
  for (int k = 0; k < count; k++) r |= (c->info[k].offs_first ? 1 : 0) | (c->info[k].offs_all ? 2 : 0);
  return r;
}

SetupLaunch setup_launch(lfvio_ctx *c, int count, int lm, bool zero_wt) {
  bool compact = count >= 8;
  for (int s = 0; compact && s < count; s++) compact = c->info[s].prior_n <= SETUP_TILED_MAXN;
  return {(compact ? 3 : SETUP_WGS) + (lm + 3) / 4, (zero_wt ? 1 : 0) | (compact ? 4 : 0)};
}

Route route_for(lfvio_ctx *c, int count, int mode) {
  Route r;
  r.count = count;
  r.g = grid_for(c, count);
  r.role_wgs = (size_t)count * (r.g.lw + (r.g.ch + 3) / 4 + LFVIO_WINDOW_SIZE + 1);
  r.split = count >= LIN_SPLIT_MIN_BATCH && r.role_wgs > LIN_SPLIT_WGS;
  bool linw = true, linb = count > 0;
  int ng = 0;
  for (int s = 0; s < count; s++) {
    linw = linw && c->info[s].linw_ok, linb = linb && c->info[s].linb_ok;
    ng = std::max(ng, c->info[s].linb_ng);
  }
  const bool solve = mode == MODE_SOLVE;
  const bool marg_sweep = (mode & (MODE_GATED - 1)) >= MODE_MARG && !(mode & (MODE_DECIDE | MODE_NOCOUNT));
  if (c->linw_mode != 0 && !c->shard_active && linw && (solve || marg_sweep) && (c->linw_mode == 2 || r.split)) r.sweep = Route::LINW;
  else if (c->linw_mode != 0 && solve && linb && (!c->shard_active || count == 1)) r.sweep = Route::LINB;
  else r.sweep = Route::ROLES;
  r.linb_gx = r.sweep == Route::LINB ? (ng + 1 + 63) / 64 * 64 : 0;
  r.setup = setup_launch(c, count, r.g.lm, r.sweep == Route::LINW);
  r.offs = slots_offs(c, count);
  return r;
}

GraphKey graph_key(const Route &r, int spec, int passes, bool with_setup) {
  GraphKey k;
  k.count = r.count, k.lm = r.g.lm, k.ch = r.g.ch, k.sc = r.g.sc, k.sweep = r.sweep, k.linb_gx = r.linb_gx, k.offs = r.offs;
  k.setup = with_setup ? r.setup.bits : 0, k.spec = spec, k.passes = passes;
  return k;
}

void launch_setup(lfvio_ctx *c, const Route &r, int mode) {
  hipLaunchKernelGGL(k_setup, dim3(r.setup.gx, r.count), dim3(256), 0, c->stream, c->d_base, c->L.total, mode, r.setup.bits);
}

template <class F>
void with_offs(bool offs, F &&launch) {
  if (offs) launch(std::true_type());
  else launch(std::false_type());
}

void launch_lin(lfvio_ctx *c, const Route &r, int mode, bool offs) {
  const int count = r.count, lw = r.g.lw, gram_wgs = (r.g.ch + 3) / 4;
  const size_t st = c->L.total;
  with_offs(offs, [&](auto o) {
    if (!r.split) {
      hipLaunchKernelGGL((k_lin<LIN_ROLE_ALL, decltype(o)::value>), dim3(lw + gram_wgs + LFVIO_WINDOW_SIZE + 1, count), dim3(LIN_THREADS), 0, c->stream, c->d_base, st,
                         mode, lw, gram_wgs);
      return;
    }
    hipLaunchKernelGGL((k_lin<LIN_ROLE_LM, decltype(o)::value>), dim3(lw, count), dim3(LIN_THREADS), 0, c->stream, c->d_base, st, mode, lw, 0);
    hipLaunchKernelGGL((k_lin<LIN_ROLE_GRAM, decltype(o)::value>), dim3(gram_wgs, count), dim3(LIN_THREADS), 0, c->stream, c->d_base, st, mode | MODE_NOCOUNT, 0, gram_wgs);
  });
  if (!r.split) return;
  const bool raw = (mode & (MODE_GATED - 1)) == MODE_SOLVE && !(mode & (MODE_GATED | MODE_DECIDE));
  if (raw) hipLaunchKernelGGL(k_imu_raw, dim3((count * LFVIO_WINDOW_SIZE + 63) / 64), dim3(64), 0, c->stream, c->d_base, st, count);
  if (raw) hipLaunchKernelGGL((k_lin<LIN_ROLE_POSE_RAW, false>), dim3(LFVIO_WINDOW_SIZE + 1, count), dim3(LIN_THREADS), 0, c->stream, c->d_base, st, mode | MODE_NOCOUNT, 0, 0);
  else hipLaunchKernelGGL((k_lin<LIN_ROLE_POSE, false>), dim3(LFVIO_WINDOW_SIZE + 1, count), dim3(LIN_THREADS), 0, c->stream, c->d_base, st, mode | MODE_NOCOUNT, 0, 0);
}

void launch_sum(lfvio_ctx *c, const Route &r, int mode) {
  const int count = r.count;
  const Grid &g = r.g;
  const size_t st = c->L.total;
  const int pre = (g.ch_raw > PRE_CHUNK_LIMIT || g.sc > 4 * PRE_GROUP) ? 1 : 0;
  const int groups = (g.sc + PRE_GROUP - 1) / PRE_GROUP;
  if (pre) hipLaunchKernelGGL(k_presum, dim3(NPAIR + (SCHUR_LEN / 256) * groups + 1, count), dim3(256), 0, c->stream, c->d_base, st, mode, groups);
  const Layout &L = c->L;
  const SumArgs sa{(long long)L.sum_off, (long long)L.sum_end_marg, (long long)L.sum_items, (long long)L.gram_part, (long long)L.pairG, (long long)L.imu_out,
                   (long long)L.prior_A};
  hipLaunchKernelGGL(k_sum, dim3(HPP_BLOCKS + SCHUR_LEN / 256 + 1, count), dim3(256), 0, c->stream, c->d_base, st, mode, pre, sa);
}

LinwArgs linw_args(const lfvio_ctx *c) {
  const Layout &L = c->L;
  LinwArgs a;
  a.anc0 = (long long)L.anc[0], a.anc_stride = (long long)(L.anc[1] - L.anc[0]);
  a.pmo0 = (long long)L.pmo[0], a.pmo_stride = (long long)(L.pmo[1] - L.pmo[0]);
  a.Wt = (long long)L.Wt, a.lam[0] = (long long)L.lam[0], a.lam[1] = (long long)L.lam[1];
  a.a = (long long)L.a, a.b = (long long)L.b, a.scale_l = (long long)L.scale_l, a.diag_l = (long long)L.diag_l, a.grad_l = (long long)L.grad_l;
  a.einv_l = (long long)L.einv_l, a.imu_out = (long long)L.imu_out;
  a.Hpp = (long long)(L.xch + (size_t)XOFF_H * 8), a.gp = (long long)(L.xch + (size_t)XOFF_G * 8), a.schur_sum = (long long)(L.xch + (size_t)XOFF_S * 8);
  a.part = (long long)L.schur_part, a.wt_ld = L.capLmBlocks * LM_BLOCK;
  a.asm_tab = c->d_lwt;
  return a;
}

void launch_sweep(lfvio_ctx *c, const Route &r, int mode, bool offs, bool decide = false) {
  if (r.sweep == Route::ROLES) {
    launch_lin(c, r, mode | (decide ? MODE_DECIDE : 0), offs);
    launch_sum(c, r, mode);
    return;
  }
  const size_t st = c->L.total;
  with_offs(offs, [&](auto o) {
    if (r.sweep == Route::LINW)
      hipLaunchKernelGGL(k_linw<decltype(o)::value>, dim3(1, r.count), dim3(LW_THREADS), LW_LDS_BYTES, c->stream, c->d_base, st, linw_args(c), mode);
    else
      hipLaunchKernelGGL(k_linb<decltype(o)::value>, dim3(r.linb_gx, r.count), dim3(LW_THREADS), LW_LDS_BYTES, c->stream, c->d_base, st, linw_args(c));
  });
  if (r.sweep == Route::LINB) hipLaunchKernelGGL(k_sumb, dim3(LINB_SUM_GRID, r.count), dim3(LINB_SUM_THREADS), 0, c->stream, c->d_base, st, linw_args(c));
}

void launch_solve(lfvio_ctx *c, int count, bool lw = false) {
  const size_t st = c->L.total;
  const long long xo = (long long)c->L.xch, io = (long long)c->L.imu_out, po = (long long)c->L.prior_A;
  if (lw)
    hipLaunchKernelGGL(k_solve_dense<true>, dim3(1, count), dim3(SOLVE_THREADS), SOLVE_LDS, c->stream, c->d_base, st, xo, io, po, (const int *)c->d_asm);
  else
    hipLaunchKernelGGL(k_solve_dense<false>, dim3(1, count), dim3(SOLVE_THREADS), SOLVE_LDS, c->stream, c->d_base, st, xo, io, po, (const int *)nullptr);
}

struct Pass {
  bool speculate = false;
  bool first = true, last = true;
  bool gauge = false;
  bool publish = false;
  bool offs = true;
};
bool launch_iteration(lfvio_ctx *c, const Route &r, int mode, const Pass &ps) {
  const int count = r.count;
  const Grid &g = r.g;
  const size_t st = c->L.total;
  const bool solve = (mode & (MODE_GATED - 1)) == MODE_SOLVE && !(mode & MODE_GATED);
  const bool lw = r.sweep == Route::LINW, lb = r.sweep == Route::LINB;
  const bool merge = solve && !lw && g.lm <= DOGLEG_INLINE_BLOCKS && r.role_wgs <= LIN_SPLIT_WGS;
  launch_sweep(c, r, mode, ps.offs, merge && !ps.first);
  if ((mode & (MODE_GATED - 1)) == MODE_SOLVE) {
    launch_solve(c, count, lw);
    const bool inl = g.lm <= DOGLEG_INLINE_BLOCKS;
    const int spec = ps.speculate && inl ? c->spec_count : 1;
    const int nb = g.lm + LFVIO_WINDOW_SIZE + 1;
    const bool split = r.split || lw;
    const bool fuse = inl && !split && !c->shard_active && (size_t)count * nb <= 2048;
    const bool stepw = lw && inl && spec == 1;
    if (stepw) {
      hipLaunchKernelGGL(k_stepw, dim3(1, count), dim3(STEPW_LAUNCH_THREADS), 0, c->stream, c->d_base, st);
      return false;
    }
    if (!inl && lb) hipLaunchKernelGGL(k_backsub_wt, dim3(g.lm, count), dim3(64), 0, c->stream, c->d_base, st, c->L.capLmBlocks * LM_BLOCK);
    else if (!inl) hipLaunchKernelGGL(k_backsub, dim3(g.lm, count), dim3(64), 0, c->stream, c->d_base, st);
// ... 53 lines not shown
  HIPCHK(c, hipGraphLaunch(graph, c->stream));
  if (int rc = behind()) return rc;
  *early = watch && wait_early(c);
  return LFVIO_OK;
}
void record_mailbox_call(lfvio_ctx *c, unsigned act) {
  record_call(c, *mail_word(c, MAIL_STATE_PASSES), ((const TRState *)(c->h_mail + MAIL_TR))->iteration, act);
}

struct LoopGraphs {
  int first_passes = 0;
  hipGraphExec_t first = nullptr, chunk = nullptr;
};
int loop_graphs(lfvio_ctx *c, const Route &r, const CallPlan &p, int passes, LoopGraphs *G) {
  const int count = r.count;
  const Grid &g = r.g;
  const bool speculate = (size_t)count * (g.lm + LFVIO_WINDOW_SIZE + 1) <= 512;
  if (speculate && !c->fixed_spec) c->spec_count = (c->last_iters > 0 && c->last_iters >= 2 * c->last_passes) ? std::min(4, 1 + SPEC_EXTRA) : 3;
  if (!c->d_pending) {
    HIPCHK(c, hipMalloc((void **)&c->d_pending, 256));
    HIPCHK(c, hipHostMalloc((void **)&c->h_pending, 256, hipHostMallocDefault));
  }
  const int offs = r.offs;
  const GraphKey key = graph_key(r, (int)speculate, 0, true);
  if (!(c->chunk_key == key)) {
    destroy_graph(c, c->chunk_key.count == count && ((c->chunk_key.offs ^ offs) & 2) == 0);
    c->chunk_key = key;
  }
  const bool fuse = p.fused;
  int first_passes = std::min(std::max(c->fixed_passes > 0 ? c->fixed_passes : c->predict_passes, 1), std::min(passes, MAX_FIRST_PASSES));
  if (p.max_seconds > 0.0) first_passes = std::max(std::min(SOLVE_CHUNK, passes), std::min(first_passes, (int)std::min(p.max_seconds / c->pass_seconds, 1e6)));
  G->first_passes = first_passes;
  const int sv = speculate && c->spec_count > 3 ? 1 : 0;
  hipGraphExec_t &first_graph = c->first[sv][p.publish ? 1 : 0][fuse ? 1 + p.marg_flag : 0][first_passes];
  enum Head { PASSES_ONLY, SETUP_FIRST };
  auto capture = [&](hipGraphExec_t *out, Head head, int npass, bool tail) {
    const bool setup = head == SETUP_FIRST;
    return capture_graph(c, c->stream, out, [&]() -> int {
      if (setup) launch_setup(c, r, MODE_SOLVE);
      bool gauged = false;
      Pass ps;
      ps.speculate = speculate, ps.gauge = tail, ps.publish = p.publish;
      for (int it = 0; it < npass; it++) {
        ps.first = it == 0, ps.last = it == npass - 1, ps.offs = (offs & 2) || (setup && it == 0 && (offs & 1));
        gauged = launch_iteration(c, r, MODE_SOLVE, ps);
      }
      if (tail) {
        if (!gauged) {
          hipLaunchKernelGGL(k_gauge, dim3(1 + (g.lm + 1) / 2, count), dim3(128), 0, c->stream, c->d_base, c->L.total, 1);
          if (p.publish) hipLaunchKernelGGL(k_publish, dim3(1), dim3(256), 0, c->stream, c->d_base, c->L.total);
        }
        if (int rc = enqueue_marg(c, p, MARG_GATED)) return rc;
      }
      if (tail && count == 1) {
        HIPCHK(c, hipMemcpyAsync(&c->h_pending->tail_state, c->d_base + offsetof(Slot, tail_state), 4 * sizeof(int), hipMemcpyDeviceToHost, c->stream));
      } else {
        hipLaunchKernelGGL(k_pending, dim3(1), dim3(64), 0, c->stream, c->d_base, c->L.total, count, c->d_pending, tail ? 1 : 0);
        HIPCHK(c, hipMemcpyAsync(&c->h_pending->open, c->d_pending, 2 * sizeof(int), hipMemcpyDeviceToHost, c->stream));
      }
      return LFVIO_OK;
    });
  };
  if (!first_graph)
    if (int rc = capture(&first_graph, SETUP_FIRST, first_passes, fuse)) return rc;
  if (!c->chunk[sv])
    if (int rc = capture(&c->chunk[sv], PASSES_ONLY, SOLVE_CHUNK,  false)) return rc;
  G->first = first_graph, G->chunk = c->chunk[sv];
  return LFVIO_OK;
}

int worker_graphs(lfvio_ctx *c, const Route &r, const CallPlan &p) {
  for (int wk = 0; wk < lfvio_ctx::WORKERS; wk++) {
    hipGraphExec_t *side_graph = &c->side[wk][p.marg_flag][p.publish ? 1 : 0];
    if (*side_graph) continue;
    hipStream_t ss = c->sstream[wk];
    const size_t back = (size_t)(c->batch + wk) * c->L.total;
    char *sh = c->d_base + back;
    const Layout &L = c->L;
    const int mode = (MODE_MARG + p.marg_flag) | MODE_GATED, gram_wgs = (L.capChunks + 3) / 4, lw_cap = 2 * DOGLEG_INLINE_BLOCKS;
    const SumArgs sa{(long long)L.sum_off - (long long)back, (long long)L.sum_end_marg - (long long)back, (long long)L.sum_items - (long long)back,
                     (long long)L.gram_part, (long long)L.pairG, (long long)L.imu_out, (long long)L.prior_A - (long long)back};
    const int rc = capture_graph(c, ss, side_graph, [&]() -> int {
      for (int rd = 0; rd < SIDE_ROUNDS; rd++) {
        hipLaunchKernelGGL(k_spec_begin, dim3(1), dim3(128), 0, ss, sh, back);
        with_offs(r.offs & 2, [&](auto o) {
          hipLaunchKernelGGL((k_lin<LIN_ROLE_ALL, decltype(o)::value>), dim3(lw_cap + gram_wgs + LFVIO_WINDOW_SIZE + 1, 1), dim3(LIN_THREADS), 0, ss, sh, back, mode,
                             lw_cap, gram_wgs);
        });
        hipLaunchKernelGGL(k_sum, dim3(HPP_BLOCKS + SCHUR_LEN / 256 + 1, 1), dim3(256), 0, ss, sh, back, mode, 0, sa);
        hipLaunchKernelGGL(k_marg_solve<true>, dim3(1, 1), dim3(MARG_THREADS), MARG_LDS, ss, sh, back,
                           p.marg_flag | (c->force_eig ? 256 : 0) | 512 | (p.publish ? 1024 : 0));
      }
      return LFVIO_OK;
    });
    if (rc) return rc;
  }
  return LFVIO_OK;
}

int adaptive_loop(lfvio_ctx *c, const Route &r, const CallPlan &p, int passes, bool *tail_done) {
  const auto t_start = std::chrono::steady_clock::now();
  LoopGraphs G;
  if (int rc = loop_graphs(c, r, p, passes, &G)) return rc;
  const int count = r.count;
  const Grid &g = r.g;
  const bool fuse = p.fused, capped = p.max_seconds > 0.0;
  const bool ahead = fuse && count == 1 && c->info[0].spec_on && c->shadow && c->marg_ahead && !c->shard_active && !c->call.pipelined() &&
                     g.lm <= DOGLEG_INLINE_BLOCKS && g.ch_raw <= PRE_CHUNK_LIMIT && g.sc <= 4 * PRE_GROUP && r.sweep == Route::ROLES;
  if (ahead)
    if (int rc = worker_graphs(c, r, p)) return rc;
  const int ticket = c->call.loop_started(ahead);
  if (c->h_mail && count == 1) *mail_word(c, MAIL_TICKET) = ticket;
  c->stat_chunks = 0;
  for (int done_passes = 0; done_passes < passes;) {
    c->stat_chunks++;
    const auto t_launch = std::chrono::steady_clock::now();
    const bool first = done_passes == 0;
    if (first) {
      bool early = false;
      const int rc = launch_watched(c, G.first, p.early && fuse && p.publish, &early, [&]() -> int {
        if (ahead) {
          for (int wk = 0; wk < lfvio_ctx::WORKERS; wk++) HIPCHK(c, hipGraphLaunch(c->side[wk][p.marg_flag][p.publish ? 1 : 0], c->sstream[wk]));
          c->call.workers_started(), c->stat_ahead_calls++;
        }
        if (c->call.pipelined()) c->up_us[1] = std::chrono::duration<double>(std::chrono::steady_clock::now() - t_launch).count() * 1e6;
        return LFVIO_OK;
      });
      if (rc) return rc;
      if (early) {
        record_mailbox_call(c, c->call.early_from_first());
        *tail_done = true;
        return LFVIO_OK;
      }
    } else
      HIPCHK(c, hipGraphLaunch(G.chunk, c->stream));
    HIPCHK(c, hipStreamSynchronize(c->stream));
    PendingBlock &hp = *c->h_pending;
    if (!first) {
      const double dt = std::chrono::duration<double>(std::chrono::steady_clock::now() - t_launch).count() / SOLVE_CHUNK;
      c->pass_seconds = 0.75 * c->pass_seconds + 0.25 * dt;
    }
    done_passes += first ? G.first_passes : SOLVE_CHUNK;
    if (first && fuse && count == 1) hp.open = hp.tail_state >= TAIL_DONE ? 0 : 1, hp.passes = hp.passes_used, c->last_iters = hp.iters_done;
    if (first && (c->call.first_graph_ended(fuse && count == 1, hp.open == 0) & CallState::CHECK_CHAIN_ERR) && hp.chain_err) {
      c->err = CHAIN_ERR_TEXT;
      return LFVIO_ERR_DEVICE;
    }
    if (hp.open == 0) {
      if (fuse && first) *tail_done = true;
      break;
    }
    if (capped && std::chrono::duration<double>(std::chrono::steady_clock::now() - t_start).count() >= p.max_seconds) {
      hipLaunchKernelGGL(k_force_done, dim3((count + 63) / 64), dim3(64), 0, c->stream, c->d_base, c->L.total, count);
      HIPCHK(c, hipStreamSynchronize(c->stream));
      break;
    }
  }
  record_call(c, c->h_pending->passes, c->last_iters, c->call.loop_ended());
  HIPCHK(c, hipGetLastError());
  if (*tail_done)
    if (int rc = wait_side(c)) return rc;
  return LFVIO_OK;
}

int enqueue_solve(lfvio_ctx *c, const CallPlan &p, bool *tail_done) {
  *tail_done = false;
  if (int rc = join_inflight(c, p.early ? CallState::OVERTAKE_PIPELINED : CallState::WAIT)) return rc;
  const Route r = route_for(c, p.count, MODE_SOLVE);
  const int passes = std::max(p.max_iter, 0) + 4;
  if (p.adaptive && c->use_graph) return adaptive_loop(c, r, p, passes, tail_done);
// ... 569 lines not shown
  mu = mu1;
  if ((rc = run(0, repeat))) return rc;
  if ((rc = run(1, full))) return rc;
  double m = 0, ref = 0;
  for (int i = 0; i < SCHUR_LEN; i++) m = std::max(m, std::fabs(repeat[i] - full[i])), ref = std::max(ref, std::fabs(full[i] - first[i]));
  *max_abs_diff = m;
  return ref > 0 ? LFVIO_OK : LFVIO_ERR_ARG;
}

int lfvio_debug_marg_system(lfvio_ctx *c, int n, double *A, double *b) {
  if (!c || !c->d_base) return LFVIO_ERR_ARG;
  (void)hipSetDevice(c->device);
  if (int rc = join_inflight(c)) return rc;
  if (n < 0 || n > 76) return LFVIO_ERR_ARG;
  if (n == 0) return LFVIO_OK;
  char *d = c->d_base + c->L.mscr;
  if (c->shadow) {
    const size_t head = offsetof(LfvioPrior, linearized_jacobians), bytes = head + sizeof(double) * n * n;
    std::vector<char> p0(bytes), pw(bytes);
    HIPCHK(c, hipMemcpy(p0.data(), c->d_base + offsetof(Slot, prior_out), bytes, hipMemcpyDeviceToHost));
    const LfvioPrior *h0 = (const LfvioPrior *)p0.data();
    for (int wk = 0; wk < lfvio_ctx::WORKERS && h0->valid == 1 && h0->n == n; wk++) {
      char *ds = c->d_base + (size_t)(c->batch + wk) * c->L.total;
      HIPCHK(c, hipMemcpy(pw.data(), ds + offsetof(Slot, prior_out), bytes, hipMemcpyDeviceToHost));
      const LfvioPrior *hw = (const LfvioPrior *)pw.data();
      if (hw->valid == 1 && hw->n == n && std::memcmp(p0.data() + head, pw.data() + head, bytes - head) == 0) {
        d = ds + c->L.mscr;
        break;
      }
    }
  }
  HIPCHK(c, hipMemcpy(A, d + sizeof(double) * (92 * 92 + 96), sizeof(double) * n * n, hipMemcpyDeviceToHost));
  HIPCHK(c, hipMemcpy(b, d + sizeof(double) * (92 * 92 + 96 + n * n), sizeof(double) * n, hipMemcpyDeviceToHost));
  return LFVIO_OK;
}

int lfvio_debug_read_clocks(lfvio_ctx *c, long long *out32) {
  if (!c || !c->d_base) return LFVIO_ERR_ARG;
  if (int rc = join_inflight(c)) return rc;
  HIPCHK(c, hipMemcpy(out32, c->d_base + offsetof(Slot, dbg), sizeof(long long) * 32, hipMemcpyDeviceToHost));
  HIPCHK(c, hipMemcpy(out32 + 32, c->d_base + offsetof(Slot, jtrace), sizeof(double) * 32, hipMemcpyDeviceToHost));
  return LFVIO_OK;
}

int lfvio_debug_time_kernel(lfvio_ctx *c, int which, int count, int reps, double *avg_ms) {
  if (!c || !c->d_base || count <= 0 || count > c->batch || reps <= 0) return LFVIO_ERR_ARG;
  (void)hipSetDevice(c->device);
  if (int rc = join_inflight(c)) return rc;
  const Route r = route_for(c, count, MODE_SOLVE);
  const Grid &g = r.g;
  const size_t st = c->L.total;
  const bool lw = r.sweep == Route::LINW, lb = r.sweep == Route::LINB;
  const bool offs = (r.offs & 2) != 0;
  if ((which == 11 || which == 12) && !lw) {
    c->err = "the resident windows are not linearized by k_linw";
    return LFVIO_ERR_ARG;
  }
  if (which >= 15 && which <= 17 && !lb) {
    c->err = "the resident window is not linearized by k_linb";
    return LFVIO_ERR_ARG;
  }
  hipEvent_t e0, e1;
  HIPCHK(c, hipEventCreate(&e0));
  if (hipError_t e = hipEventCreate(&e1); e != hipSuccess) {
    (void)hipEventDestroy(e0);
    HIPCHK(c, e);
  }
  launch_setup(c, r, MODE_SOLVE);
  Route full = r;
  if (lb && !(which >= 15 && which <= 17)) full.sweep = Route::ROLES;
  launch_sweep(c, full, MODE_SOLVE, offs);
  if (which == 14) launch_solve(c, count, lw);
  if (which == 17) launch_solve(c, count, false);

  HIPCHK(c, hipEventRecord(e0, c->stream));
  for (int rep = 0; rep < reps; rep++) {
    switch (which) {
      case 0: launch_lin(c, r, MODE_SOLVE, offs); break;
      case 2: launch_sum(c, r, MODE_SOLVE); break;
      case 8: case 9: case 10: case 18: {
        const int gram_wgs = (g.ch + 3) / 4;
        const int gx = which == 8 ? g.lw : which == 9 ? gram_wgs : which == 18 ? LFVIO_WINDOW_SIZE : LFVIO_WINDOW_SIZE + 1;
        hipLaunchKernelGGL((k_lin<LIN_ROLE_ALL, false>), dim3(gx, count), dim3(LIN_THREADS), 0, c->stream, c->d_base, st, MODE_SOLVE, which == 8 ? g.lw : 0,
                           which == 9 ? gram_wgs : 0);
      } break;
      case 4: case 5: case 6: case 7: {
        const SetupLaunch sl = setup_launch(c, count, g.lm, false);
        const int wgs = (sl.bits & 4) ? 3 : SETUP_WGS, gx = which == 4 ? 1 : which == 5 ? 2 : which == 6 ? wgs : sl.gx;
        hipLaunchKernelGGL(k_setup, dim3(gx, count), dim3(256), 0, c->stream, c->d_base, st, MODE_SOLVE, sl.bits);
      } break;
      case 11: case 12: launch_sweep(c, r, MODE_SOLVE, offs); break;
      case 13: launch_solve(c, count, lw); break;
      case 14: hipLaunchKernelGGL(k_stepw, dim3(1, count), dim3(STEPW_LAUNCH_THREADS), 0, c->stream, c->d_base, st); break;
      case 15: hipLaunchKernelGGL(k_linb<false>, dim3(r.linb_gx, count), dim3(LW_THREADS), LW_LDS_BYTES, c->stream, c->d_base, st, linw_args(c)); break;
      case 16: hipLaunchKernelGGL(k_sumb, dim3(LINB_SUM_GRID, count), dim3(LINB_SUM_THREADS), 0, c->stream, c->d_base, st, linw_args(c)); break;
      case 17: hipLaunchKernelGGL(k_backsub_wt, dim3(g.lm, count), dim3(64), 0, c->stream, c->d_base, st, c->L.capLmBlocks * LM_BLOCK); break;
      default: launch_solve(c, count); break;
    }
  }
  HIPCHK(c, hipEventRecord(e1, c->stream));
  HIPCHK(c, hipEventSynchronize(e1));
  float ms = 0;
  HIPCHK(c, hipEventElapsedTime(&ms, e0, e1));
  *avg_ms = (double)ms / reps;
  (void)hipEventDestroy(e0);
  (void)hipEventDestroy(e1);
  return LFVIO_OK;
}

static int sweep_kernel_of(lfvio_ctx *c, int count) {
  return !c || !c->d_base || count <= 0 || count > c->batch ? LFVIO_ERR_ARG : route_for(c, count, MODE_SOLVE).sweep;
}

int lfvio_debug_resident_pass(lfvio_ctx *c, int count, int slot, double *gp, double *schur, double *lm_sum, double *a, double *b, double *gn_p, double *q,
                              double *x_cost) {
  if (!c || !c->d_base || count <= 0 || count > c->batch || slot < 0 || slot >= count) return LFVIO_ERR_ARG;
  (void)hipSetDevice(c->device);
  if (int rc = join_inflight(c)) return rc;
  for (int s = 0; s < count; s++)
    if (!c->info[s].resident) return LFVIO_ERR_ARG;
  const size_t st = c->L.total;
  const Route r = route_for(c, count, MODE_SOLVE);
  launch_setup(c, r, MODE_SOLVE);
  launch_sweep(c, r, MODE_SOLVE, true);
  launch_solve(c, count, r.sweep == Route::LINW);
  HIPCHK(c, hipGetLastError());
  HIPCHK(c, hipStreamSynchronize(c->stream));
  const char *d = c->d_base + (size_t)slot * st;
  const int N = c->info[slot].N;
  auto get = [&](double *dst, size_t off, size_t n) { return !dst || !n ? hipSuccess : hipMemcpy(dst, d + off, n * 8, hipMemcpyDeviceToHost); };
  HIPCHK(c, get(gp, c->L.xch + (size_t)XOFF_G * 8, KP));
  HIPCHK(c, get(schur, c->L.xch + (size_t)XOFF_S * 8, SCHUR_LEN));
  HIPCHK(c, get(lm_sum, offsetof(Slot, lm_sum), 5));
  HIPCHK(c, get(a, c->L.a, N));
  HIPCHK(c, get(b, c->L.b, N));
  HIPCHK(c, get(gn_p, offsetof(Slot, gn_p), KP));
  HIPCHK(c, get(q, offsetof(Slot, tr) + offsetof(TRState, q), Q_COUNT));
  HIPCHK(c, get(x_cost, offsetof(Slot, tr) + offsetof(TRState, x_cost), 1));
  return r.sweep;
}

int lfvio_debug_configure(lfvio_ctx *c, const char *key, double value) {
  if (!c || !key) return LFVIO_ERR_ARG;
  const std::string k = key;
  const int iv = (int)value;
  if (k == "env") {
    const char *e = getenv("LFVIO_DEBUG");
    if (!e) return LFVIO_OK;
    std::string all = e;
    for (size_t p = 0; p < all.size();) {
      const size_t q = std::min(all.find(',', p), all.size()), eq = all.find('=', p);
      if (eq != std::string::npos && eq < q) {
        const int rc = lfvio_debug_configure(c, all.substr(p, eq - p).c_str(), atof(all.substr(eq + 1, q - eq - 1).c_str()));
        if (rc) return rc;
      }
      p = q + 1;
    }
    return LFVIO_OK;
  }
  const bool structural = k == "graph" || k == "linw" || k == "force_eig";
  if (structural) {
    if (int rc = join_inflight(c)) return rc;
  }
  if (k == "graph") c->use_graph = iv != 0;
  else if (k == "first_passes") {
    if (iv < 0) return LFVIO_ERR_ARG;
    c->fixed_passes = iv;
// ... 55 lines not shown
```

### lf-vio_amd/csrc/tr_decide.h

```cpp
#pragma once
#include "dev_math.h"
#include "dev_types.h"

DEV double pick_cand(double first, const double (&e)[SPEC_EXTRA], int z) {
  double v = first;
#pragma unroll
  for (int j = 0; j < SPEC_EXTRA; j++) v = z == j + 1 ? e[j] : v;
  return v;
}
DEV double pick_slot(const double (&a)[1 + SPEC_EXTRA], int z) {
  double v = a[0];
#pragma unroll
  for (int j = 1; j < 1 + SPEC_EXTRA; j++) v = z == j ? a[j] : v;
  return v;
}

DEV TRFlags tr_flags_decided(const Slot *S) {
  TRFlags f = tr_flags(&S->tr);
  const int pending = S->dec_pending;
  const int it = S->dec.iteration, cur = S->dec.cur, dl = S->dec.do_lin, ds = S->dec.do_schur, dn = S->dec.done, te = S->dec.termination, cf = S->dec.chol_fail;
  if (pending) f.iteration = it, f.cur = cur, f.do_lin = dl, f.do_schur = ds, f.done = dn, f.termination = te, f.chol_fail = cf;
  return f;
}

DEV void tr_init(TRState *t, double radius, double function_tolerance) {
  t->radius = radius;
  t->function_tolerance = function_tolerance;
  t->mu = 1e-8;
  t->x_cost = t->cand_cost = t->model_cost_change = t->dogleg_step_norm = t->alpha = 0.0;
  t->iteration = 0;
  t->cur = 0;
  t->do_lin = 1;
  t->do_schur = 1;
  t->done = 0;
  t->termination = LFVIO_NO_CONVERGENCE;
  t->chol_fail = 0;
  t->scaled = 0;
  t->num_succ = t->num_unsucc = t->consec_invalid = t->trace_len = 0;
  t->step_valid = 0;
  t->skip_step = 0;
  t->error = 0;
  t->new_point = 0;
  t->spec_n = 1;
}

struct DecideSums {
  double cost[1 + SPEC_EXTRA], mlin[1 + SPEC_EXTRA], mquad[1 + SPEC_EXTRA], dn[1 + SPEC_EXTRA], xn[1 + SPEC_EXTRA];
};
DEV int decide_candidates(const TRHead &t) { return t.chol_fail ? 1 : (t.spec_n < 1 ? 1 : (t.spec_n > 1 + SPEC_EXTRA ? 1 + SPEC_EXTRA : t.spec_n)); }

DEV void decide_sums(const Slot *S, const TRHead &t, int K, int sharded, int nLmBlocks, int lane, DecideSums &o) {
  const double *cp0 = S->cost_part, *cpE = S->cost_partE, *pc0 = S->pose_cost;
  double c[1 + SPEC_EXTRA], l[1 + SPEC_EXTRA], q[1 + SPEC_EXTRA], d[1 + SPEC_EXTRA], x[1 + SPEC_EXTRA];
#pragma unroll
  for (int z = 0; z < 1 + SPEC_EXTRA; z++) {
    const double *cp = z == 0 ? cp0 : cpE + (size_t)(z > 0 ? z - 1 : 0) * (SPEC_MAX_LM / 64) * LMS;
    const double *pcz = z == 0 ? pc0 : (const double *)S->pose_costE[z > 0 ? z - 1 : 0];
    const int nbz = z == 0 ? nLmBlocks : min(nLmBlocks, SPEC_MAX_LM / 64);
    c[z] = l[z] = q[z] = d[z] = x[z] = 0.0;
#pragma unroll 8
    for (int k = lane; k < nbz; k += 64) {
      const double *p = cp + (size_t)k * LMS;
      c[z] += p[0], l[z] += p[1], q[z] += p[2], d[z] += p[3], x[z] += p[4];
    }
    if (lane < 11) c[z] += pcz[lane];
  }
#pragma unroll
  for (int z = 0; z < 1 + SPEC_EXTRA; z++) {
    const bool use = !t.chol_fail && z < K && !sharded;
    o.cost[z] = use ? wave_sum(c[z]) : 0.0, o.mlin[z] = use ? wave_sum(l[z]) : 0.0, o.mquad[z] = use ? wave_sum(q[z]) : 0.0;
    o.dn[z] = use ? wave_sum(d[z]) : 0.0, o.xn[z] = use ? wave_sum(x[z]) : 0.0;
  }
  if (sharded && !t.chol_fail) {
    const double *sc = S->xch + XOFF_C;
    o.cost[0] = sc[XS_CCOST], o.mlin[0] = sc[XS_MLIN], o.mquad[0] = sc[XS_MQUAD], o.dn[0] = sc[XS_DN], o.xn[0] = sc[XS_XN];
  }
}

DEV int decide_walk(TRHead &t, const DecideSums &sm, int K, int sharded, int max_iter, TRState *trace_dst) {
  int acc_z = 0;
  if (t.chol_fail && t.mu < 1.0) {
    t.do_lin = sharded ? 1 : 0;
    t.do_schur = 1;
    t.chol_fail = 0;
    t.skip_step = 1;
    return 0;
  }
  const double function_tolerance = t.function_tolerance, gradient_tolerance = 1e-10, parameter_tolerance = 1e-8;
  const double min_relative_decrease = 1e-3, min_trust_region_radius = 1e-32;
  (void)gradient_tolerance;
  for (int z = 0; z < K; z++) {
    const double cgz = pick_cand(t.cg, t.cgE, z), cnz = pick_cand(t.cn, t.cnE, z), snz = pick_cand(t.dogleg_step_norm, t.snE, z);
    const double step_sq = pick_cand(t.step_sq_pose, t.step_sqE, z), xn2c = pick_cand(t.xn2_pose_cand, t.xn2E, z);
    const double cost_z = pick_slot(sm.cost, z), mlin_z = pick_slot(sm.mlin, z), mquad_z = pick_slot(sm.mquad, z), dn_z = pick_slot(sm.dn, z), xn_z = pick_slot(sm.xn, z);
    LfvioIterationSummary it;
    it.cost = t.x_cost, it.cost_change = 0, it.gradient_max_norm = 0, it.step_norm = 0, it.relative_decrease = 0;
    it.step_is_valid = 0, it.step_is_successful = 0;
    bool finished = false, go_on = false;
    bool step_valid = false;
    double model_cost_change = 0;
    if (!t.chol_fail) {
      const double lin = cgz * t.q[Q_gG] + cnz * t.q[Q_gN] + mlin_z;
      const double quad = cgz * cgz * t.q[Q_GG] + 2.0 * cgz * cnz * t.q[Q_GN] + cnz * cnz * t.q[Q_NN] + mquad_z;
      model_cost_change = -lin - 0.5 * quad;
      step_valid = model_cost_change > 0.0;
    }
    t.model_cost_change = model_cost_change;
    it.step_is_valid = step_valid ? 1 : 0;
    if (!step_valid) {
      if (++t.consec_invalid >= 5) {
        t.termination = LFVIO_FAILURE;
        t.done = 1;
        finished = true;
      } else {
        t.mu *= 10.0;
        t.chol_fail = 0;
        t.do_lin = sharded ? 1 : 0;
        t.do_schur = 1;
      }
    } else {
      t.consec_invalid = 0;
      const double candidate_cost = isfinite(cost_z) ? cost_z : 1.79769313486231570815e+308;
      t.cand_cost = candidate_cost;
      it.step_norm = sqrt(step_sq + dn_z);
      if (it.step_norm <= parameter_tolerance * (t.x_norm + parameter_tolerance)) {
        t.termination = LFVIO_CONVERGENCE;
        t.done = 1;
        finished = true;
      } else {
        it.cost_change = t.x_cost - candidate_cost;
        if (fabs(it.cost_change) <= function_tolerance * t.x_cost) {
          t.termination = LFVIO_CONVERGENCE;
          t.done = 1;
          finished = true;
        } else {
          it.relative_decrease = it.cost_change / model_cost_change;
          if (it.relative_decrease > min_relative_decrease) {
            t.cur ^= 1;
            acc_z = z;
            t.x_norm = sqrt(xn2c + xn_z);
            it.step_is_successful = 1;
            it.cost = candidate_cost;
            it.gradient_max_norm = __builtin_nan("");
            if (it.relative_decrease < 0.25) t.radius *= 0.5;
            if (it.relative_decrease > 0.75) t.radius = fmax(t.radius, 3.0 * snz);
            t.mu = fmax(1e-8, 2.0 * t.mu / 10.0);
            t.do_lin = 1;
            t.do_schur = 1;
            t.x_cost = candidate_cost;
          } else {
            t.radius *= 0.5;
            t.do_lin = 0;
            t.do_schur = 0;
            it.cost = candidate_cost;
            go_on = true;
          }
        }
      }
    }
// ... 59 lines not shown
```

Baseline: 2412 solves/s.

## Pass slot array offsets as kernel args and hoist first loads before gating

Introduces a SlotArgs struct of precomputed byte offsets passed by value to k_lin and k_spec_begin, so kernels can compute input addresses without first reading GP pointers from the slot. Each block issues its first-round loads (landmark metadata, chunk bounds, prior J, cost partials for the decide step) at kernel entry, speculatively and with clamped indices, before the trust-region gate and decision logic. This is meant to overlap dependent global-memory latency with the decision phase. The cost is extra register pressure, and loads are wasted when a block exits early.

New measurement: 2447 solves/s (median of 6 runs). 1.5% higher.

```diff
diff --git a/lf-vio_amd/csrc/dev_types.h b/lf-vio_amd/csrc/dev_types.h
--- a/lf-vio_amd/csrc/dev_types.h
+++ b/lf-vio_amd/csrc/dev_types.h
@@ -18,6 +18,7 @@
 constexpr int PRE_CHUNK_LIMIT = 2 * 121;
 constexpr int SUM_ITEMS_CAP = PRE_CHUNK_LIMIT * 209 + 64;
 constexpr int SUM_VIS_PACKED = 73 * 74 / 2, SUM_VIS = SUM_VIS_PACKED + 73;
+constexpr int LINB_LEN = SUM_VIS + SCHUR_LEN + 8;
 constexpr int HPP_CAP = 16384;
 constexpr int XOFF_H = 0;
 constexpr int XOFF_G = 14880;
diff --git a/lf-vio_amd/csrc/kernels_lin.h b/lf-vio_amd/csrc/kernels_lin.h
--- a/lf-vio_amd/csrc/kernels_lin.h
+++ b/lf-vio_amd/csrc/kernels_lin.h
@@ -1,10 +1,21 @@
 #pragma once
 #include "dev_factors.h"
+#include "slot_args.h"
 #include "kernels_spec.h"
 #include "tr_decide.h"
 #include <type_traits>
 
 #define SLOT(base, stride) ((Slot *)((char *)(base) + (size_t)blockIdx.y * (stride)))
+template <class T>
+DEV T *blob_at(const Slot *S, long long off) { return (T *)((char *)S + off); }
+DEV void load_obs(const Slot *S, const SlotArgs &A, int o, d3 &p, d3 &v, double &td, double &row) {
+  const char *c0 = (const char *)S + A.obs0;
+  auto ch = [&](int k) { return ((const double *)(c0 + k * A.obs_stride))[o]; };
+  p = mk3(ch(0), ch(1), ch(2));
+  v = mk3(ch(3), ch(4), ch(5));
+  td = ch(6);
+  row = ch(7);
+}
 
 constexpr int MODE_SOLVE = 0;
 constexpr int MODE_MARG = 1;
@@ -367,8 +378,27 @@
 #else
 #define LSTAMP(k) do { } while (0)
 #endif
+constexpr int LIN_ROLE_LM = 1, LIN_ROLE_GRAM = 2, LIN_ROLE_POSE = 4, LIN_ROLE_ALL = 7;
+struct LinFirst {
+  int st, cnt, obs0, woff;
+  int ch_pair, ch_begin, ch_end;
+};
+template <int ROLES>
+DEV void lin_first(const Slot *S, const SlotArgs &A, int gLw, int gCh, int half, LinFirst &F) {
+  const int b = blockIdx.x, tid = threadIdx.x;
+  if ((ROLES & LIN_ROLE_LM) && b < gLw) {
+    const int *st = blob_at<int>(S, A.lm_start), *cnt = blob_at<int>(S, A.lm_cnt), *o0 = blob_at<int>(S, A.lm_obs0), *wo = blob_at<int>(S, A.lm_woff);
+    const int l4 = first_lm_in_index(A, b * LM_BLOCK + tid / 4), l8 = first_lm_in_index(A, b * (LM_BLOCK / 2) + tid / 8);
+    const int s4 = st[l4], c4 = cnt[l4], o4 = o0[l4], w4 = wo[l4], s8 = st[l8], c8 = cnt[l8], o8 = o0[l8], w8 = wo[l8];
+    F.st = half ? s8 : s4, F.cnt = half ? c8 : c4, F.obs0 = half ? o8 : o4, F.woff = half ? w8 : w4;
+  } else if ((ROLES & LIN_ROLE_GRAM) && b >= gLw && b - gLw < gCh) {
+    const int chunk = first_chunk_index(A, 4 * (b - gLw) + (tid >> 6));
+    F.ch_pair = blob_at<int>(S, A.chunk_pair)[chunk], F.ch_begin = blob_at<int>(S, A.chunk_begin)[chunk], F.ch_end = blob_at<int>(S, A.chunk_end)[chunk];
+  }
+}
+
 template <bool TIGHT, int LPT, bool OFFS>
-DEV void lin_landmark_role(Slot *S, const LinView &lv, int wg, int mode, double *lds, double *part) {
+DEV void lin_landmark_role(Slot *S, const SlotArgs &A, const LinFirst &F, const LinView &lv, int wg, int mode, double *lds, double *part) {
   constexpr int LMB = LIN_THREADS / LPT;
   double(*tile)[WLD + 1] = (double(*)[WLD + 1]) lds;
   double *red = lds + LM_BLOCK * (WLD + 1);
@@ -391,17 +421,17 @@
   d3 wPi = mk3(0, 0, 0), wTi = wPi, wTic = wPi, wTx = wPi;
   int i = 0, cnt_l = 0, woff_l = 0;
   if (valid) {
-    i = S->lm_start[l];
-    const int k = S->lm_cnt[l], o0 = S->lm_obs0[l];
-    cnt_l = k, woff_l = S->lm_woff[l];
+    i = F.st;
+    const int k = F.cnt, o0 = F.obs0;
+    cnt_l = k, woff_l = F.woff;
     lam = lv.lam[l];
     ObsPair ob;
-    load_obs(S, o0, ob.pi, ob.vi, ob.tdi, ob.rowi);
+    load_obs(S, A, o0, ob.pi, ob.vi, ob.tdi, ob.rowi);
     const m33 ricT = ldm(T->ricT);
     const unsigned offm = OFFS ? tab_offmask(T) : 0u;
     for (int o = 1 + q; o < k; o += LPT) {
       const int j = i + o, pair = i * 11 + j;
-      load_obs(S, o0 + o, ob.pj, ob.vj, ob.tdj, ob.rowj);
+      load_obs(S, A, o0 + o, ob.pj, ob.vj, ob.tdj, ob.rowj);
       PairU u;
       if (OFFS) load_pair_uniform(T, pair, offm, u);
       else load_pair_uniform(T, pair, u);
@@ -520,7 +550,7 @@
 }
 
 template <bool OFFS>
-DEV void lin_gram_role(Slot *S, const LinView &lv, int wg, int mode, double *lds) {
+DEV void lin_gram_role(Slot *S, const SlotArgs &A, const LinFirst &F, const LinView &lv, int wg, int mode, double *lds) {
   const int wv = threadIdx.x >> 6, lane = threadIdx.x & 63;
   const int chunk = 4 * wg + wv;
   if (chunk >= S->nChunks) return;
@@ -531,9 +561,9 @@
   double(*E)[20] = (double(*)[20])(my + 32 * 17 + 256);
   double(*T1)[20] = (double(*)[20]) my;
   const Tab *T = lv.tab;
-  const int pair = S->chunk_pair[chunk];
+  const int pair = F.ch_pair;
   const int j = pair % 11;
-  const int begin = S->chunk_begin[chunk], end = S->chunk_end[chunk];
+  const int begin = F.ch_begin, end = F.ch_end;
   const int est_td = S->est_td;
   const double td = lv.x->td;
   PairU u;
@@ -546,12 +576,12 @@
 #pragma unroll
   for (int e = 0; e < 14; e++) c0[e] = c1[e] = 0.0;
   if (idx < end) {
-    const int oj = S->pm_obs[idx], l = S->pm_lm[idx];
-    const int oi = S->lm_obs0[l];
+    const int oj = blob_at<int>(S, A.pm_obs)[idx], l = blob_at<int>(S, A.pm_lm)[idx];
+    const int oi = blob_at<int>(S, A.lm_obs0)[l];
     const double lam = lv.lam[l];
     ObsPair ob;
-    load_obs(S, oi, ob.pi, ob.vi, ob.tdi, ob.rowi);
-    load_obs(S, oj, ob.pj, ob.vj, ob.tdj, ob.rowj);
+    load_obs(S, A, oi, ob.pi, ob.vi, ob.tdi, ob.rowi);
+    load_obs(S, A, oj, ob.pj, ob.vj, ob.tdj, ob.rowj);
     Basis B;
     visual_basis<OFFS>(ob, lam, td, est_td, S->tr_over_row, S->half_row, S->sqrt_info, u, B);
     c0[0] = B.red[0].x, c0[1] = B.red[0].y, c0[2] = B.red[0].z;
@@ -677,8 +707,10 @@
   }
 }
 
+constexpr int LIN_PRIOR_PER = (LIN_PRIOR_N * LIN_PRIOR_N + LIN_THREADS - 1) / LIN_THREADS;
+static_assert(LIN_PRIOR_PER * LIN_THREADS == FIRST_PRIOR_J, "the speculative rounds of J0 are the ones slot_args.h accounts for");
 template <bool STAGED>
-DEV void lin_prior_role(Slot *S, const LinView &lv, int mode, double *lds) {
+DEV void lin_prior_role(Slot *S, const double *Jg, const double *prior_r, const double *jfirst, const LinView &lv, int mode, double *lds) {
   const int n = S->prior_n;
   const bool staged = STAGED && n <= LIN_PRIOR_N;
   double *Js = lds, *dx = lds + (STAGED ? LIN_PRIOR_N * LIN_PRIOR_N : 0), *r = dx + KP, *part = r + KP;
@@ -687,12 +719,11 @@
   for (int c = tid; c < KP + 4; c += LIN_THREADS) g[c] = 0.0;
   if (!S->prior_valid || (S->sharded && !S->pose_side)) return;
   const FrameState *x = lv.x;
-  const double *Jg = S->prior_J;
   if (staged) {
-    constexpr int PER = (LIN_PRIOR_N * LIN_PRIOR_N + LIN_THREADS - 1) / LIN_THREADS;
+    constexpr int PER = LIN_PRIOR_PER;
     double v[PER];
 #pragma unroll
-    for (int k = 0; k < PER; k++) v[k] = tid + LIN_THREADS * k < n * n ? Jg[tid + LIN_THREADS * k] : 0.0;
+    for (int k = 0; k < PER; k++) v[k] = tid + LIN_THREADS * k < n * n ? jfirst[k] : 0.0;
     if (tid < S->prior_nb) prior_block_dx(S, x, tid, dx);
 #pragma unroll
     for (int k = 0; k < PER; k++)
@@ -706,7 +737,7 @@
     double s = 0;
     for (int c = tid & 3; c < n; c += 4) s = fma(J[row * n + c], dx[c], s);
     s = quad_sum(s);
-    if ((tid & 3) == 0) r[row] = S->prior_r[row] + s;
+    if ((tid & 3) == 0) r[row] = prior_r[row] + s;
   }
   __syncthreads();
   {
@@ -742,11 +773,10 @@
   imu_raw_jacobian(&S->imu[f], S->g, x->pose[f], x->sb[f], x->pose[f + 1], x->sb[f + 1], raw);
 }
 
-constexpr int LIN_ROLE_LM = 1, LIN_ROLE_GRAM = 2, LIN_ROLE_POSE = 4, LIN_ROLE_ALL = 7;
 constexpr int LIN_ROLE_POSE_RAW = 8;
 constexpr int LIN_LDS_POSE = 1024;
 template <int ROLES, bool OFFS = true>
-__global__ __launch_bounds__(LIN_THREADS, ROLES == LIN_ROLE_GRAM ? 3 : (ROLES == LIN_ROLE_POSE_RAW ? 6 : 2)) void k_lin(char *base, size_t stride, int mode_bits, int gLw, int gCh) {
+__global__ __launch_bounds__(LIN_THREADS, ROLES == LIN_ROLE_GRAM ? 3 : (ROLES == LIN_ROLE_POSE_RAW ? 6 : 2)) void k_lin(char *base, size_t stride, int mode_bits, int gLw, int gCh, const SlotArgs A) {
   Slot *S = SLOT(base, stride);
   TRState *tr = &S->tr;
   const int mode = mode_bits & (MODE_GATED - 1);
@@ -755,20 +785,40 @@
   int do_lin = fl.do_lin, do_schur = fl.do_schur, cur = fl.cur, acc_z = 0;
   double mu = tr->mu;
   int num_succ = tr->num_succ;
+  const int N = S->N, half = S->lm_half, tail_state = S->tail_state;
+  LinFirst F;
+  lin_first<ROLES>(S, A, gLw, gCh, half, F);
+  constexpr bool STAGED_PRIOR = ROLES == LIN_ROLE_ALL;
+  double jfirst[LIN_PRIOR_PER];
+  if (STAGED_PRIOR && (int)blockIdx.x == gLw + gCh + LFVIO_WINDOW_SIZE) {
+    const double *Jg = blob_at<double>(S, A.prior_J);
+#pragma unroll
+    for (int k = 0; k < LIN_PRIOR_PER; k++) jfirst[k] = Jg[threadIdx.x + LIN_THREADS * k];
+  }
+  const bool decide = ROLES == LIN_ROLE_ALL && (mode_bits & MODE_DECIDE) && !(mode_bits & MODE_GATED);
+  TRHead t;
+  DecideFirst df;
+  int nLmBlocks = 0, max_iter = 0, spec_on = 0;
+  if (decide) {
+    nLmBlocks = S->nLmBlocks, max_iter = S->max_iter, spec_on = S->spec_on;
+    if (threadIdx.x < 64) {
+      t = *reinterpret_cast<const TRHead *>(tr);
+      decide_first(S, threadIdx.x, blob_at<double>(S, A.cost_part), blob_at<double>(S, A.cost_partE), A.cap_blocks, df);
+    }
+  }
   if (mode_bits & MODE_GATED) {
-    if (!tail_gate(S, fl.done)) return;
+    if (!(fl.done && tail_state == TAIL_OPEN)) return;
   } else {
     int done = fl.done;
     const bool owner = blockIdx.x == 0 && !(mode_bits & MODE_NOCOUNT);
-    if ((mode_bits & MODE_DECIDE) && !done) {
+    if (decide && !done) {
       __shared__ TRDecision dsh;
       if (threadIdx.x < 64) {
-        TRHead t = *reinterpret_cast<const TRHead *>(tr);
         const int K = decide_candidates(t);
         DecideSums sm;
-        decide_sums(S, t, K, 0, S->nLmBlocks, threadIdx.x, sm);
+        decide_sums(S, t, K, 0, nLmBlocks, threadIdx.x, sm, blob_at<double>(S, A.cost_part), blob_at<double>(S, A.cost_partE), &df);
         if (threadIdx.x == 0) {
-          const int az = decide_walk(t, sm, K, 0, S->max_iter, owner ? tr : nullptr);
+          const int az = decide_walk(t, sm, K, 0, max_iter, owner ? tr : nullptr);
           decision_from(dsh, t, az);
           if (owner) S->dec = dsh, S->dec_pending = 1;
         }
@@ -779,13 +829,13 @@
       num_succ = __builtin_amdgcn_readfirstlane(dsh.num_succ);
       mu = __hiloint2double(__builtin_amdgcn_readfirstlane(__double2hiint(dsh.mu)), __builtin_amdgcn_readfirstlane(__double2loint(dsh.mu)));
       if (acc_z > 0 && blockIdx.x == gridDim.x - 1 && !(mode_bits & MODE_NOCOUNT)) {
-        copy_accepted(S, acc_z, cur, S->N, threadIdx.x, LIN_THREADS);
-        if (S->spec_on) {
+        copy_accepted(S, acc_z, cur, N, threadIdx.x, LIN_THREADS);
+        if (spec_on) {
           __threadfence();
           __syncthreads();
           if (threadIdx.x == 0) spec_publish(S, num_succ, cur);
         }
-      } else if (acc_z == 0 && owner && threadIdx.x == 0 && S->spec_on) spec_publish(S, num_succ, cur);
+      } else if (acc_z == 0 && owner && threadIdx.x == 0 && spec_on) spec_publish(S, num_succ, cur);
     } else if (owner && threadIdx.x == 0 && mode == MODE_SOLVE && S->spec_on) spec_publish(S, num_succ, cur);
     if (mode == MODE_SOLVE && owner && !done && threadIdx.x == 0) S->passes_used++;
     if (done | (!do_lin & !do_schur)) return;
@@ -799,15 +849,15 @@
   int b = blockIdx.x;
   if (b < gLw) {
     if (ROLES & LIN_ROLE_LM) {
-      const int half = S->lm_half, lmb = half ? LM_BLOCK / 2 : LM_BLOCK;
-      const int nblk = ((is_marg(mode) ? marg_plan(S, mode)->N0 : S->N) + lmb - 1) / lmb;
+      const int lmb = half ? LM_BLOCK / 2 : LM_BLOCK;
+      const int nblk = ((is_marg(mode) ? marg_plan(S, mode)->N0 : N) + lmb - 1) / lmb;
       if (b >= nblk) return;
       double *part = S->schur_part + (size_t)b * SCHUR_LEN;
       if (half) {
-        if (do_lin) lin_landmark_role<ROLES == LIN_ROLE_ALL, 8, OFFS>(S, lv, b, mode, lds, part);
+        if (do_lin) lin_landmark_role<ROLES == LIN_ROLE_ALL, 8, OFFS>(S, A, F, lv, b, mode, lds, part);
         else lin_schur_only_role<8>(S, lv, b, lds, part);
       } else {
-        if (do_lin) lin_landmark_role<ROLES == LIN_ROLE_ALL, 4, OFFS>(S, lv, b, mode, lds, part);
+        if (do_lin) lin_landmark_role<ROLES == LIN_ROLE_ALL, 4, OFFS>(S, A, F, lv, b, mode, lds, part);
         else lin_schur_only_role<4>(S, lv, b, lds, part);
       }
     }
@@ -816,7 +866,7 @@
   if (!do_lin) return;
   b -= gLw;
   if (b < gCh) {
-    if (ROLES & LIN_ROLE_GRAM) lin_gram_role<OFFS>(S, lv, b, mode, lds);
+    if (ROLES & LIN_ROLE_GRAM) lin_gram_role<OFFS>(S, A, F, lv, b, mode, lds);
     return;
   }
   b -= gCh;
@@ -826,7 +876,7 @@
       else lin_imu_role<false>(S, lv, b, mode, lds);
       return;
     }
-    lin_prior_role<ROLES == LIN_ROLE_ALL>(S, lv, mode, lds);
+    lin_prior_role<STAGED_PRIOR>(S, STAGED_PRIOR ? blob_at<double>(S, A.prior_J) : (double *)S->prior_J, S->prior_r, jfirst, lv, mode, lds);
   }
 }
 
@@ -939,8 +989,6 @@
 struct SumArgs {
   long long sum_off, sum_end_marg, sum_items, gram_part, pairG, imu_out, prior_A;
 };
-template <class T>
-DEV T *blob_at(const Slot *S, long long off) { return (T *)((char *)S + off); }
 #define SUM_KEEP(v) asm volatile("" ::"v"(v))
 
 DEV void sum_hpp_entry(Slot *S, const SumArgs &o, int mode_bits, int e) {
diff --git a/lf-vio_amd/csrc/kernels_linw.h b/lf-vio_amd/csrc/kernels_linw.h
--- a/lf-vio_amd/csrc/kernels_linw.h
+++ b/lf-vio_amd/csrc/kernels_linw.h
@@ -434,7 +434,7 @@
   const int tid = threadIdx.x;
   const int n = S->prior_n;
   if (!S->prior_valid || (S->sharded && !S->pose_side) || n > LW_PRIOR_MAXN) {
-    lin_prior_role<false>(S, lv, MODE_SOLVE, lw);
+    lin_prior_role<false>(S, S->prior_J, S->prior_r, nullptr, lv, MODE_SOLVE, lw);
     __syncthreads();
     return;
   }
@@ -761,7 +761,6 @@
   linw_body<OFFS>(SLOT(base, stride), lw, A, mode_bits);
 }
 
-constexpr int LINB_LEN = SUM_VIS + SCHUR_LEN + 8;
 __global__ __launch_bounds__(256) void k_linb_gather(char *base, size_t stride) {
   Slot *S = SLOT(base, stride);
   if (!S->linw.big) return;
diff --git a/lf-vio_amd/csrc/kernels_marg.h b/lf-vio_amd/csrc/kernels_marg.h
--- a/lf-vio_amd/csrc/kernels_marg.h
+++ b/lf-vio_amd/csrc/kernels_marg.h
@@ -224,7 +224,7 @@
   const long long t0 = wall_clock64();
   while (spec_peek(&S->tail_state) == TAIL_WORKER && wall_clock64() - t0 < 10 * SPEC_WAIT_TICKS) __builtin_amdgcn_s_sleep(8);
 }
-__global__ __launch_bounds__(128) void k_spec_begin(char *base, size_t back) {
+__global__ __launch_bounds__(128) void k_spec_begin(char *base, size_t back, const SlotArgs A) {
   Slot *S = (Slot *)base;
   Slot *S0 = (Slot *)(base - back);
   const int tid = threadIdx.x;
@@ -275,8 +275,8 @@
       static_assert(TW <= 128, "the trust-region header in one trip");
       const double *xs = (const double *)&S0->x[cur];
       double *xd = (double *)&S->x[0];
-      const double *ls = S0->lam[cur];
-      double *ld = S->lam[0];
+      const double *ls = blob_at<const double>(S0, cur ? A.lam[1] : A.lam[0]);
+      double *ld = blob_at<double>(S, A.lam[0]);
       const int N = S0->N;
       const long long *ts = (const long long *)&S0->tr;
       long long *td = (long long *)&S->tr;
@@ -284,7 +284,7 @@
 #pragma unroll
       for (int k = 0; k < XT; k++) xv[k] = xs[tid + 128 * k < XW ? tid + 128 * k : 0];
 #pragma unroll
-      for (int k = 0; k < LT; k++) lv[k] = ls[tid + 128 * k < N ? tid + 128 * k : 0];
+      for (int k = 0; k < LT; k++) lv[k] = ls[first_lm_index(A, tid + 128 * k)];
       const long long tv = ts[tid < TW ? tid : 0];
 #pragma unroll
       for (int k = 0; k < XT; k++)
diff --git a/lf-vio_amd/csrc/lfvio_hip.hip b/lf-vio_amd/csrc/lfvio_hip.hip
--- a/lf-vio_amd/csrc/lfvio_hip.hip
+++ b/lf-vio_amd/csrc/lfvio_hip.hip
@@ -48,74 +48,6 @@
 
 namespace {
 
-inline size_t align_up(size_t v, size_t a) { return (v + a - 1) / a * a; }
-
-struct Layout {
-  int maxN = 0, maxM = 0;
-  int capLmBlocks = 0, capChunks = 0, capSchurParts = 0;
-  size_t in_begin = 0, in_end = 0, total = 0;
-  size_t anc[8], pmo[8], pm_pair, linb_lm0, linb_ns, linw_begin = 0, linw_end = 0;
-  size_t lm_start, lm_cnt, lm_obs0, lm_perm, lm_woff, lam0, obs[8], pm_obs, pm_lm, chunk_pair, chunk_begin, chunk_end, sum_off, sum_end_marg, sum_items, prior_J,
-      prior_r;
-  size_t lam[2], lamE[SPEC_EXTRA], cost_partE, prior_A, a, b, W, Wt, scale_l, grad_l, gn_l, diag_l, einv_l, d1, d2, gram_part, pairG, schur_part,
-      xch, lm_part, cost_part, imu_out, imu_raw, mscr, eig_aux;
-};
-
-Layout make_layout(int maxN, int maxM) {
-  Layout L;
-  L.maxN = maxN;
-  L.maxM = maxM;
-  L.capLmBlocks = std::max(1, (maxN + LM_BLOCK - 1) / LM_BLOCK);
-  L.capChunks = 64 + maxM / CHUNK_MAX;
-  L.capSchurParts = std::max(L.capLmBlocks + 1, 2 * ((std::min(maxN, SPEC_MAX_LM) + LM_BLOCK - 1) / LM_BLOCK));
-  static_assert(LINB_LEN >= SCHUR_LEN, "the Schur partials of k_lin share the array of k_linb's group partials, which are the larger");
-  size_t o = align_up(sizeof(Slot), 256);
-  auto take = [&](size_t bytes) {
-    size_t r = o;
-    o = align_up(o + bytes, 256);
-    return r;
-  };
-  const size_t N = std::max(maxN, 1), M = std::max(maxM, 1), LB = (size_t)L.capLmBlocks * LM_BLOCK;
-  L.in_begin = o;
-  L.lm_start = take(N * 4), L.lm_cnt = take(N * 4), L.lm_obs0 = take(N * 4), L.lm_perm = take(N * 4);
-  L.lm_woff = take((N + 1) * 4);
-  L.lam0 = take(N * 8);
-  for (int k = 0; k < 8; k++) L.obs[k] = take(M * 8);
-  L.pm_obs = take(M * 4), L.pm_lm = take(M * 4);
-  L.chunk_pair = take((size_t)L.capChunks * 4), L.chunk_begin = take((size_t)L.capChunks * 4),
-  L.chunk_end = take((size_t)L.capChunks * 4);
-  L.prior_r = take(LFVIO_MAX_PRIOR_DIM * 8);
-  L.sum_off = take((size_t)(SUM_VIS + 1) * 4), L.sum_end_marg = take((size_t)SUM_VIS * 4);
-  L.sum_items = take((size_t)SUM_ITEMS_CAP * 4);
-  L.prior_J = take((size_t)LFVIO_MAX_PRIOR_DIM * LFVIO_MAX_PRIOR_DIM * 8);
-  L.in_end = o;
-  L.linw_begin = o;
-  for (int k = 0; k < 8; k++) L.anc[k] = take(N * 8);
-  for (int k = 0; k < 8; k++) L.pmo[k] = take(M * 8);
-  L.pm_pair = take(M);
-  L.linb_lm0 = take(((size_t)L.capLmBlocks + LFVIO_NUM_FRAMES + 1) * 4), L.linb_ns = take(((size_t)L.capLmBlocks + LFVIO_NUM_FRAMES + 1) * 4);
-  L.linw_end = o;
-  L.lam[0] = take(LB * 8), L.lam[1] = take(LB * 8);
-  for (int k = 0; k < SPEC_EXTRA; k++) L.lamE[k] = take((size_t)SPEC_MAX_LM * 8);
-  L.cost_partE = take((size_t)SPEC_EXTRA * (SPEC_MAX_LM / 64) * LMS * 8);
-  L.prior_A = take((size_t)LFVIO_MAX_PRIOR_DIM * LFVIO_MAX_PRIOR_DIM * 8);
-  L.a = take(LB * 8), L.b = take(LB * 8), L.W = take(LB * WLD * 8);
-  L.Wt = take((size_t)WT_PAIRS * std::max((size_t)SPEC_MAX_LM, LB) * 16);
-  L.scale_l = take(LB * 8), L.grad_l = take(LB * 8), L.gn_l = take(LB * 8), L.diag_l = take(LB * 8);
-  L.einv_l = take(LB * 8), L.d1 = take(LB * 8), L.d2 = take(LB * 8);
-  L.gram_part = take((size_t)L.capChunks * NGP * 8);
-  L.pairG = take((size_t)NPAIR * NGP * 8);
-  L.schur_part = take((size_t)L.capSchurParts * LINB_LEN * 8);
-  L.xch = take((size_t)XCH_ALLOC * 8);
-  L.lm_part = take((size_t)L.capLmBlocks * LMS * 8);
-  L.cost_part = take((size_t)L.capLmBlocks * LMS * 8);
-  L.imu_out = take((size_t)LFVIO_WINDOW_SIZE * IMU_OUT * 8);
-  L.imu_raw = take((size_t)LFVIO_WINDOW_SIZE * IMU_RAW * 8);
-  L.mscr = take((size_t)HPP_CAP * 8);
-  L.eig_aux = take(4096);
-  L.total = align_up(o, 4096);
-  return L;
-}
 
 size_t down_bytes(int maxN) { return sizeof(FrameState) * 2 + sizeof(TRState) + 2 * ((size_t)maxN * 8 + 128) + sizeof(LfvioPrior) + 4096; }
 
@@ -1035,20 +967,21 @@
 void launch_lin(lfvio_ctx *c, const Route &r, int mode, bool offs) {
   const int count = r.count, lw = r.g.lw, gram_wgs = (r.g.ch + 3) / 4;
   const size_t st = c->L.total;
+  const SlotArgs sa = slot_args(c->L);
   with_offs(offs, [&](auto o) {
     if (!r.split) {
       hipLaunchKernelGGL((k_lin<LIN_ROLE_ALL, decltype(o)::value>), dim3(lw + gram_wgs + LFVIO_WINDOW_SIZE + 1, count), dim3(LIN_THREADS), 0, c->stream, c->d_base, st,
-                         mode, lw, gram_wgs);
+                         mode, lw, gram_wgs, sa);
       return;
     }
-    hipLaunchKernelGGL((k_lin<LIN_ROLE_LM, decltype(o)::value>), dim3(lw, count), dim3(LIN_THREADS), 0, c->stream, c->d_base, st, mode, lw, 0);
-    hipLaunchKernelGGL((k_lin<LIN_ROLE_GRAM, decltype(o)::value>), dim3(gram_wgs, count), dim3(LIN_THREADS), 0, c->stream, c->d_base, st, mode | MODE_NOCOUNT, 0, gram_wgs);
+    hipLaunchKernelGGL((k_lin<LIN_ROLE_LM, decltype(o)::value>), dim3(lw, count), dim3(LIN_THREADS), 0, c->stream, c->d_base, st, mode, lw, 0, sa);
+    hipLaunchKernelGGL((k_lin<LIN_ROLE_GRAM, decltype(o)::value>), dim3(gram_wgs, count), dim3(LIN_THREADS), 0, c->stream, c->d_base, st, mode | MODE_NOCOUNT, 0, gram_wgs, sa);
   });
   if (!r.split) return;
   const bool raw = (mode & (MODE_GATED - 1)) == MODE_SOLVE && !(mode & (MODE_GATED | MODE_DECIDE));
   if (raw) hipLaunchKernelGGL(k_imu_raw, dim3((count * LFVIO_WINDOW_SIZE + 63) / 64), dim3(64), 0, c->stream, c->d_base, st, count);
-  if (raw) hipLaunchKernelGGL((k_lin<LIN_ROLE_POSE_RAW, false>), dim3(LFVIO_WINDOW_SIZE + 1, count), dim3(LIN_THREADS), 0, c->stream, c->d_base, st, mode | MODE_NOCOUNT, 0, 0);
-  else hipLaunchKernelGGL((k_lin<LIN_ROLE_POSE, false>), dim3(LFVIO_WINDOW_SIZE + 1, count), dim3(LIN_THREADS), 0, c->stream, c->d_base, st, mode | MODE_NOCOUNT, 0, 0);
+  if (raw) hipLaunchKernelGGL((k_lin<LIN_ROLE_POSE_RAW, false>), dim3(LFVIO_WINDOW_SIZE + 1, count), dim3(LIN_THREADS), 0, c->stream, c->d_base, st, mode | MODE_NOCOUNT, 0, 0, sa);
+  else hipLaunchKernelGGL((k_lin<LIN_ROLE_POSE, false>), dim3(LFVIO_WINDOW_SIZE + 1, count), dim3(LIN_THREADS), 0, c->stream, c->d_base, st, mode | MODE_NOCOUNT, 0, 0, sa);
 }
 
 void launch_sum(lfvio_ctx *c, const Route &r, int mode) {
@@ -1268,10 +1201,10 @@
                      (long long)L.gram_part, (long long)L.pairG, (long long)L.imu_out, (long long)L.prior_A - (long long)back};
     const int rc = capture_graph(c, ss, side_graph, [&]() -> int {
       for (int rd = 0; rd < SIDE_ROUNDS; rd++) {
-        hipLaunchKernelGGL(k_spec_begin, dim3(1), dim3(128), 0, ss, sh, back);
+        hipLaunchKernelGGL(k_spec_begin, dim3(1), dim3(128), 0, ss, sh, back, slot_args(L));
         with_offs(r.offs & 2, [&](auto o) {
           hipLaunchKernelGGL((k_lin<LIN_ROLE_ALL, decltype(o)::value>), dim3(lw_cap + gram_wgs + LFVIO_WINDOW_SIZE + 1, 1), dim3(LIN_THREADS), 0, ss, sh, back, mode,
-                             lw_cap, gram_wgs);
+                             lw_cap, gram_wgs, slot_args(L, back));
         });
         hipLaunchKernelGGL(k_sum, dim3(HPP_BLOCKS + SCHUR_LEN / 256 + 1, 1), dim3(256), 0, ss, sh, back, mode, 0, sa);
         hipLaunchKernelGGL(k_marg_solve<true>, dim3(1, 1), dim3(MARG_THREADS), MARG_LDS, ss, sh, back,
@@ -2007,7 +1940,7 @@
         const int gram_wgs = (g.ch + 3) / 4;
         const int gx = which == 8 ? g.lw : which == 9 ? gram_wgs : which == 18 ? LFVIO_WINDOW_SIZE : LFVIO_WINDOW_SIZE + 1;
         hipLaunchKernelGGL((k_lin<LIN_ROLE_ALL, false>), dim3(gx, count), dim3(LIN_THREADS), 0, c->stream, c->d_base, st, MODE_SOLVE, which == 8 ? g.lw : 0,
-                           which == 9 ? gram_wgs : 0);
+                           which == 9 ? gram_wgs : 0, slot_args(c->L));
       } break;
       case 4: case 5: case 6: case 7: {
         const SetupLaunch sl = setup_launch(c, count, g.lm, false);
diff --git a/lf-vio_amd/csrc/slot_args.h b/lf-vio_amd/csrc/slot_args.h
--- /dev/null
+++ b/lf-vio_amd/csrc/slot_args.h
@@ -0,0 +1,139 @@
+#pragma once
+#if !defined(__HIPCC__) && !defined(__host__)
+#define __host__
+#define __device__
+#define __forceinline__ inline
+#endif
+#include <algorithm>
+#include <cstddef>
+#include "dev_types.h"
+
+inline size_t align_up(size_t v, size_t a) { return (v + a - 1) / a * a; }
+
+struct Layout {
+  int maxN = 0, maxM = 0;
+  int capLmBlocks = 0, capChunks = 0, capSchurParts = 0;
+  size_t in_begin = 0, in_end = 0, total = 0;
+  size_t anc[8], pmo[8], pm_pair, linb_lm0, linb_ns, linw_begin = 0, linw_end = 0;
+  size_t lm_start, lm_cnt, lm_obs0, lm_perm, lm_woff, lam0, obs[8], pm_obs, pm_lm, chunk_pair, chunk_begin, chunk_end, sum_off, sum_end_marg, sum_items, prior_J,
+      prior_r;
+  size_t lam[2], lamE[SPEC_EXTRA], cost_partE, prior_A, a, b, W, Wt, scale_l, grad_l, gn_l, diag_l, einv_l, d1, d2, gram_part, pairG, schur_part,
+      xch, lm_part, cost_part, imu_out, imu_raw, mscr, eig_aux;
+};
+
+inline Layout make_layout(int maxN, int maxM) {
+  Layout L;
+  L.maxN = maxN;
+  L.maxM = maxM;
+  L.capLmBlocks = std::max(1, (maxN + LM_BLOCK - 1) / LM_BLOCK);
+  L.capChunks = 64 + maxM / CHUNK_MAX;
+  L.capSchurParts = std::max(L.capLmBlocks + 1, 2 * ((std::min(maxN, SPEC_MAX_LM) + LM_BLOCK - 1) / LM_BLOCK));
+  static_assert(LINB_LEN >= SCHUR_LEN, "the Schur partials of k_lin share the array of k_linb's group partials, which are the larger");
+  size_t o = align_up(sizeof(Slot), 256);
+  auto take = [&](size_t bytes) {
+    size_t r = o;
+    o = align_up(o + bytes, 256);
+    return r;
+  };
+  const size_t N = std::max(maxN, 1), M = std::max(maxM, 1), LB = (size_t)L.capLmBlocks * LM_BLOCK;
+  L.in_begin = o;
+  L.lm_start = take(N * 4), L.lm_cnt = take(N * 4), L.lm_obs0 = take(N * 4), L.lm_perm = take(N * 4);
+  L.lm_woff = take((N + 1) * 4);
+  L.lam0 = take(N * 8);
+  for (int k = 0; k < 8; k++) L.obs[k] = take(M * 8);
+  L.pm_obs = take(M * 4), L.pm_lm = take(M * 4);
+  L.chunk_pair = take((size_t)L.capChunks * 4), L.chunk_begin = take((size_t)L.capChunks * 4),
+  L.chunk_end = take((size_t)L.capChunks * 4);
+  L.prior_r = take(LFVIO_MAX_PRIOR_DIM * 8);
+  L.sum_off = take((size_t)(SUM_VIS + 1) * 4), L.sum_end_marg = take((size_t)SUM_VIS * 4);
+  L.sum_items = take((size_t)SUM_ITEMS_CAP * 4);
+  L.prior_J = take((size_t)LFVIO_MAX_PRIOR_DIM * LFVIO_MAX_PRIOR_DIM * 8);
+  L.in_end = o;
+  L.linw_begin = o;
+  for (int k = 0; k < 8; k++) L.anc[k] = take(N * 8);
+  for (int k = 0; k < 8; k++) L.pmo[k] = take(M * 8);
+  L.pm_pair = take(M);
+  L.linb_lm0 = take(((size_t)L.capLmBlocks + LFVIO_NUM_FRAMES + 1) * 4), L.linb_ns = take(((size_t)L.capLmBlocks + LFVIO_NUM_FRAMES + 1) * 4);
+  L.linw_end = o;
+  L.lam[0] = take(LB * 8), L.lam[1] = take(LB * 8);
+  for (int k = 0; k < SPEC_EXTRA; k++) L.lamE[k] = take((size_t)SPEC_MAX_LM * 8);
+  L.cost_partE = take((size_t)SPEC_EXTRA * (SPEC_MAX_LM / 64) * LMS * 8);
+  L.prior_A = take((size_t)LFVIO_MAX_PRIOR_DIM * LFVIO_MAX_PRIOR_DIM * 8);
+  L.a = take(LB * 8), L.b = take(LB * 8), L.W = take(LB * WLD * 8);
+  L.Wt = take((size_t)WT_PAIRS * std::max((size_t)SPEC_MAX_LM, LB) * 16);
+  L.scale_l = take(LB * 8), L.grad_l = take(LB * 8), L.gn_l = take(LB * 8), L.diag_l = take(LB * 8);
+  L.einv_l = take(LB * 8), L.d1 = take(LB * 8), L.d2 = take(LB * 8);
+  L.gram_part = take((size_t)L.capChunks * NGP * 8);
+  L.pairG = take((size_t)NPAIR * NGP * 8);
+  L.schur_part = take((size_t)L.capSchurParts * LINB_LEN * 8);
+  L.xch = take((size_t)XCH_ALLOC * 8);
+  L.lm_part = take((size_t)L.capLmBlocks * LMS * 8);
+  L.cost_part = take((size_t)L.capLmBlocks * LMS * 8);
+  L.imu_out = take((size_t)LFVIO_WINDOW_SIZE * IMU_OUT * 8);
+  L.imu_raw = take((size_t)LFVIO_WINDOW_SIZE * IMU_RAW * 8);
+  L.mscr = take((size_t)HPP_CAP * 8);
+  L.eig_aux = take(4096);
+  L.total = align_up(o, 4096);
+  return L;
+}
+
+struct SlotArgs {
+  long long lm_start, lm_cnt, lm_obs0, lm_woff;
+  long long obs0, obs_stride;
+  long long pm_obs, pm_lm;
+  long long chunk_pair, chunk_begin, chunk_end;
+  long long prior_J;
+  long long lam[2];
+  long long cost_part, cost_partE;
+  int cap_lm_in, cap_chunks, cap_blocks, cap_lm;
+};
+constexpr int SLOT_INPUT_OFFSETS = 12;
+
+__host__ __device__ inline int first_clamp(int i, int cap) { return i < cap ? i : cap - 1; }
+__host__ __device__ inline int first_lm_in_index(const SlotArgs &A, int l) { return first_clamp(l, A.cap_lm_in); }
+__host__ __device__ inline int first_chunk_index(const SlotArgs &A, int c) { return first_clamp(c, A.cap_chunks); }
+__host__ __device__ inline int first_lm_index(const SlotArgs &A, int l) { return first_clamp(l, A.cap_lm); }
+__host__ __device__ inline int first_block_index(int cap_blocks, int lane) { return first_clamp(lane, cap_blocks); }
+__host__ __device__ inline int first_blockE_index(int cap_blocks, int lane) { return first_clamp(lane, cap_blocks < SPEC_MAX_LM / 64 ? cap_blocks : SPEC_MAX_LM / 64); }
+constexpr int FIRST_PRIOR_J = ((76 * 76 + 255) / 256) * 256;
+static_assert(FIRST_PRIOR_J <= LFVIO_MAX_PRIOR_DIM * LFVIO_MAX_PRIOR_DIM, "the speculative rounds of J0 stay inside the array");
+
+inline SlotArgs slot_args(const Layout &L, size_t back = 0) {
+  SlotArgs A;
+  const long long bk = (long long)back;
+  A.lm_start = (long long)L.lm_start - bk, A.lm_cnt = (long long)L.lm_cnt - bk, A.lm_obs0 = (long long)L.lm_obs0 - bk, A.lm_woff = (long long)L.lm_woff - bk;
+  A.obs0 = (long long)L.obs[0] - bk, A.obs_stride = (long long)(L.obs[1] - L.obs[0]);
+  A.pm_obs = (long long)L.pm_obs - bk, A.pm_lm = (long long)L.pm_lm - bk;
+  A.chunk_pair = (long long)L.chunk_pair - bk, A.chunk_begin = (long long)L.chunk_begin - bk, A.chunk_end = (long long)L.chunk_end - bk;
+  A.prior_J = (long long)L.prior_J - bk;
+  A.lam[0] = (long long)L.lam[0], A.lam[1] = (long long)L.lam[1];
+  A.cost_part = (long long)L.cost_part, A.cost_partE = (long long)L.cost_partE;
+  A.cap_lm_in = std::max(L.maxN, 1), A.cap_chunks = L.capChunks, A.cap_blocks = L.capLmBlocks, A.cap_lm = L.capLmBlocks * LM_BLOCK;
+  return A;
+}
+
+struct SlotArgSpan {
+  const char *name;
+  long long off, bytes, array;
+  int input;
+};
+constexpr int SLOT_ARG_SPANS = 15;
+inline int slot_arg_spans(const Layout &L, const SlotArgs &A, SlotArgSpan *out) {
+  int n = 0;
+  auto put = [&](const char *name, long long off, long long bytes, long long array, int input) { out[n++] = SlotArgSpan{name, off, bytes, array, input}; };
+  constexpr int BIG = 0x7fffffff;
+  const long long N = std::max(L.maxN, 1), M = std::max(L.maxM, 1), LB = (long long)L.capLmBlocks * LM_BLOCK;
+  const long long lin = (first_lm_in_index(A, BIG) + 1) * 4ll, ch = (first_chunk_index(A, BIG) + 1) * 4ll;
+  put("lm_start", A.lm_start, lin, N * 4, 1), put("lm_cnt", A.lm_cnt, lin, N * 4, 1), put("lm_obs0", A.lm_obs0, lin, N * 4, 1);
+  put("lm_woff", A.lm_woff, lin, (N + 1) * 4, 1);
+  put("obs0", A.obs0, 7 * A.obs_stride + 8, 7 * A.obs_stride + M * 8, 1);
+  put("pm_obs", A.pm_obs, 4, M * 4, 1), put("pm_lm", A.pm_lm, 4, M * 4, 1);
+  put("chunk_pair", A.chunk_pair, ch, (long long)L.capChunks * 4, 1), put("chunk_begin", A.chunk_begin, ch, (long long)L.capChunks * 4, 1);
+  put("chunk_end", A.chunk_end, ch, (long long)L.capChunks * 4, 1);
+  put("prior_J", A.prior_J, (long long)FIRST_PRIOR_J * 8, (long long)LFVIO_MAX_PRIOR_DIM * LFVIO_MAX_PRIOR_DIM * 8, 1);
+  put("lam0", A.lam[0], (first_lm_index(A, BIG) + 1) * 8ll, LB * 8, 0), put("lam1", A.lam[1], (first_lm_index(A, BIG) + 1) * 8ll, LB * 8, 0);
+  put("cost_part", A.cost_part, (first_block_index(A.cap_blocks, BIG) + 1ll) * LMS * 8, (long long)L.capLmBlocks * LMS * 8, 0);
+  put("cost_partE", A.cost_partE, ((long long)(SPEC_EXTRA - 1) * (SPEC_MAX_LM / 64) + first_blockE_index(A.cap_blocks, BIG) + 1) * LMS * 8,
+      (long long)SPEC_EXTRA * (SPEC_MAX_LM / 64) * LMS * 8, 0);
+  return n;
+}
diff --git a/lf-vio_amd/csrc/tr_decide.h b/lf-vio_amd/csrc/tr_decide.h
--- a/lf-vio_amd/csrc/tr_decide.h
+++ b/lf-vio_amd/csrc/tr_decide.h
@@ -1,6 +1,7 @@
 #pragma once
 #include "dev_math.h"
 #include "dev_types.h"
+#include "slot_args.h"
 
 DEV double pick_cand(double first, const double (&e)[SPEC_EXTRA], int z) {
   double v = first;
@@ -49,21 +50,36 @@
 };
 DEV int decide_candidates(const TRHead &t) { return t.chol_fail ? 1 : (t.spec_n < 1 ? 1 : (t.spec_n > 1 + SPEC_EXTRA ? 1 + SPEC_EXTRA : t.spec_n)); }
 
-DEV void decide_sums(const Slot *S, const TRHead &t, int K, int sharded, int nLmBlocks, int lane, DecideSums &o) {
-  const double *cp0 = S->cost_part, *cpE = S->cost_partE, *pc0 = S->pose_cost;
-  double c[1 + SPEC_EXTRA], l[1 + SPEC_EXTRA], q[1 + SPEC_EXTRA], d[1 + SPEC_EXTRA], x[1 + SPEC_EXTRA];
+struct DecideFirst {
+  double f[1 + SPEC_EXTRA][5], pc[1 + SPEC_EXTRA];
+};
+DEV void decide_first(const Slot *S, int lane, const double *cp0, const double *cpE, int cap, DecideFirst &o) {
 #pragma unroll
   for (int z = 0; z < 1 + SPEC_EXTRA; z++) {
     const double *cp = z == 0 ? cp0 : cpE + (size_t)(z > 0 ? z - 1 : 0) * (SPEC_MAX_LM / 64) * LMS;
-    const double *pcz = z == 0 ? pc0 : (const double *)S->pose_costE[z > 0 ? z - 1 : 0];
+    const double *pcz = z == 0 ? (const double *)S->pose_cost : (const double *)S->pose_costE[z > 0 ? z - 1 : 0];
+    const double *p = cp + (size_t)(z == 0 ? first_block_index(cap, lane) : first_blockE_index(cap, lane)) * LMS;
+#pragma unroll
+    for (int e = 0; e < 5; e++) o.f[z][e] = p[e];
+    o.pc[z] = pcz[lane < 11 ? lane : 0];
+  }
+}
+DEV void decide_sums(const Slot *S, const TRHead &t, int K, int sharded, int nLmBlocks, int lane, DecideSums &o, const double *cp0, const double *cpE, const DecideFirst *first) {
+  double c[1 + SPEC_EXTRA], l[1 + SPEC_EXTRA], q[1 + SPEC_EXTRA], d[1 + SPEC_EXTRA], x[1 + SPEC_EXTRA];
+#pragma unroll
+  for (int z = 0; z < 1 + SPEC_EXTRA; z++) {
+    const double *cp = z == 0 ? cp0 : cpE + (size_t)(z > 0 ? z - 1 : 0) * (SPEC_MAX_LM / 64) * LMS;
     const int nbz = z == 0 ? nLmBlocks : min(nLmBlocks, SPEC_MAX_LM / 64);
+    const double *pcz = z == 0 ? (const double *)S->pose_cost : (const double *)S->pose_costE[z > 0 ? z - 1 : 0];
+    const bool in = lane < nbz;
     c[z] = l[z] = q[z] = d[z] = x[z] = 0.0;
+    if (first) c[z] += in ? first->f[z][0] : 0.0, l[z] += in ? first->f[z][1] : 0.0, q[z] += in ? first->f[z][2] : 0.0, d[z] += in ? first->f[z][3] : 0.0, x[z] += in ? first->f[z][4] : 0.0;
 #pragma unroll 8
-    for (int k = lane; k < nbz; k += 64) {
+    for (int k = first ? lane + 64 : lane; k < nbz; k += 64) {
       const double *p = cp + (size_t)k * LMS;
       c[z] += p[0], l[z] += p[1], q[z] += p[2], d[z] += p[3], x[z] += p[4];
     }
-    if (lane < 11) c[z] += pcz[lane];
+    if (lane < 11) c[z] += first ? first->pc[z] : pcz[lane];
   }
 #pragma unroll
   for (int z = 0; z < 1 + SPEC_EXTRA; z++) {
@@ -75,6 +91,10 @@
     const double *sc = S->xch + XOFF_C;
     o.cost[0] = sc[XS_CCOST], o.mlin[0] = sc[XS_MLIN], o.mquad[0] = sc[XS_MQUAD], o.dn[0] = sc[XS_DN], o.xn[0] = sc[XS_XN];
   }
+}
+
+DEV void decide_sums(const Slot *S, const TRHead &t, int K, int sharded, int nLmBlocks, int lane, DecideSums &o) {
+  decide_sums(S, t, K, sharded, nLmBlocks, lane, o, S->cost_part, S->cost_partE, nullptr);
 }
 
 DEV int decide_walk(TRHead &t, const DecideSums &sm, int K, int sharded, int max_iter, TRState *trace_dst) {
```
